# nikhilTkur/Multigrid_Nikhil_C-

Hardware: AMD Instinct MI355X
Metric: fine_grid_stencil_updates_per_sec (higher is better)
Workload: dtype f64

## Files before the change

### multigrid_nikhil_c-_amd/csrc/mgx.hip

```cpp

#include "../../include/mgx.h"
#include "mgx_bottom.hpp"
#include "mgx_kernels.hpp"
#include "mgx_launch.hpp"
#include "mgx_var.hpp"
#include "mgx_galerkin.hpp"
#include "mgx_opdep.hpp"
#include "mgx_cheby.hpp"
#include "mgx_line.hpp"
#include "mgx_colour.hpp"
#include "mgx_small.hpp"
#include "mgx_krylov.hpp"
#include "mgx_refine.hpp"
#include "mgx_refine_gcr.hpp"
#include "mgx_multi.hpp"
#include "mgx_eig.hpp"
#include "mgx_eig_many.hpp"
#include "mgx_theta.hpp"
#include "mgx_newton.hpp"
#include "mgx_dist_plan.hpp"

#include <chrono>
#include <unistd.h>
#include <cmath>
// ... 370 lines not shown
}

int lambda_update(mgx_solver* s, Level& l)
{
    if (l.f64) launch_lambda_max<double>(var_level<double>(l), s->partial, s->partial_cap, s->sum_dev, s->stream);
    else launch_lambda_max<float>(var_level<float>(l), s->partial, s->partial_cap, s->sum_dev, s->stream);
    HIPCHK(s, hipGetLastError());
    HIPCHK(s, hipMemcpyAsync(s->sum_host, s->sum_dev, sizeof(double), hipMemcpyDeviceToHost, s->stream));
    HIPCHK(s, hipStreamSynchronize(s->stream));
    l.lambda_g = *s->sum_host;
    return MGX_OK;
}

template <typename T> LineLevel<T> line_level(const Level& l)
{
    return LineLevel<T>{op9_of<T>(l), l.nine, l.N, l.pitch, (T*)l.line_m[0], (T*)l.line_g[0], (T*)l.line_m[1], (T*)l.line_g[1],
                        (T*)l.line_hf, (T*)l.line_hb, l.line_R};
}

int line_update(mgx_solver* s, Level& l)
{
    if (!s->line_dirs) return MGX_OK;
    HIPCHK(s, hipMemsetAsync(s->line_flag, 0, sizeof(int), s->stream));
    for (int d = 0; d < 2; ++d) {
        if (!(s->line_dirs & (1 << d))) continue;
        if (l.f64) launch_line_factor<double>(line_level<double>(l), d, s->line_flag, s->stream);
        else launch_line_factor<float>(line_level<float>(l), d, s->line_flag, s->stream);
    }
    HIPCHK(s, hipGetLastError());
    int flag = 0;
    HIPCHK(s, hipMemcpyAsync(&flag, s->line_flag, sizeof(int), hipMemcpyDeviceToHost, s->stream));
    HIPCHK(s, hipStreamSynchronize(s->stream));
    if (flag)
        return s->fail(MGX_ERR_INVALID, "MGX_SMOOTHER_LINE: zero or non-finite pivot in the tridiagonal factorisation of level " +
                                            std::to_string(l.L) + ", direction " + ((flag & 1) ? "x" : "y"));
    return MGX_OK;
}

template <typename T>
void build_splitting(mgx_solver* s, const Level& l)
{
    const dim3 blk(256), grd((l.N + 1 + 255) / 256, l.N + 1);
    with_point_count(l.nine, [&](auto nq) {
        hipLaunchKernelGGL((k_var_build_jacobi<T, decltype(nq)::value>), grd, blk, 0, s->stream, op9_of<T>(l), out9(jac9_of<T>(l)), l.N, l.pitch,
                           (T)s->cfg.omega);
    });
}
template <typename T>
void build_bottom_inverse(mgx_solver* s, const Level& l)
{
    const int n = l.N - 1, NN = n * n;
    with_point_count(l.nine, [&](auto nq) {
        hipLaunchKernelGGL((k_var_dense_fill<T, decltype(nq)::value>), dim3((NN + 255) / 256, NN), dim3(256), 0, s->stream, s->var_M, s->var_inv,
                           op9_of<T>(l), n, l.pitch);
    });
    gj_invert(s, NN);
}

template <typename T>
int var_build_t(mgx_solver* s, Level& l)
{
    build_splitting<T>(s, l);
    if (l.L == s->cfg.coarsest_level && s->cfg.bottom == MGX_BOTTOM_EXACT) build_bottom_inverse<T>(s, l);
    HIPCHK(s, hipGetLastError());
    HIPCHK(s, hipStreamSynchronize(s->stream));
    if (int rc = lambda_update(s, l)) return rc;
    if (int rc = line_update(s, l)) { l.stencil_set = false; operator_changed(s); return rc; }
    l.stencil_set = true;
    operator_changed(s);
    return MGX_OK;
}
int var_build(mgx_solver* s, Level& l) { return l.f64 ? var_build_t<double>(s, l) : var_build_t<float>(s, l); }

template <typename T> Wt8<T> wt8_of(const Level& c)
{
    Wt8<T> w;
    for (int x = 0; x < 8; ++x) w.w[x] = (const T*)c.wt[x];
    return w;
}
template <typename T> Wt8Out<T> wt8_out(const Level& c)
{
    Wt8Out<T> w;
    for (int x = 0; x < 8; ++x) w.w[x] = (T*)c.wt[x];
    return w;
}

inline bool opdep(const mgx_solver* s) { return s->galerkin && s->gal_built && s->transfer == MGX_TRANSFER_OPERATOR; }

template <typename T>
int galerkin_build_t(mgx_solver* s, int transfer)
{
    const int lo = s->cfg.coarsest_level, hi = s->cfg.finest_level;
    const T rscale = (s->cfg.restrict_mode == MGX_RESTRICT_FW16) ? (T)0.25 : (T)1;
    if (transfer == MGX_TRANSFER_OPERATOR)
        for (int lv = lo; lv < hi; ++lv)
            for (void*& p : s->lv[lv].wt) {
                if (p) continue;
                if (hipMalloc(&p, s->lv[lv].bytes) != hipSuccess) return s->fail(MGX_ERR_ALLOC, "hipMalloc failed for the prolongation's weight arrays");
                HIPCHK(s, hipMemsetAsync(p, 0, s->lv[lv].bytes, s->stream));
            }
    for (int lv = hi; lv > lo; --lv) {
        const Level& f = s->lv[lv];
        const Level& c = s->lv[lv - 1];
        const Launch g = make_launch(c.N, VecOf<T>::W, c.N - 1, 1);
        const dim3 grd(g.blocks), blk(kBlock);
        with_point_count(f.nine, [&](auto nq) {
            constexpr bool CORNERS = decltype(nq)::value == 9;
            if (transfer == MGX_TRANSFER_OPERATOR) {
                hipLaunchKernelGGL((k_opdep_weights<T, CORNERS>), grd, blk, 0, s->stream, op9_of<T>(f), wt8_out<T>(c), c.N, f.pitch, c.pitch, g.strips);
                hipLaunchKernelGGL((k_galerkin_rap_opdep<T, CORNERS>), grd, blk, 0, s->stream, op9_of<T>(f), wt8_of<T>(c), out9(op9_of<T>(c)), c.N,
                                   f.pitch, c.pitch, g.strips, rscale);
            }
            else hipLaunchKernelGGL((k_galerkin_rap<T, CORNERS>), grd, blk, 0, s->stream, op9_of<T>(f), out9(op9_of<T>(c)), c.N, f.pitch, c.pitch,
                                    g.strips, rscale);
        });
    }
    for (int lv = lo; lv <= hi; ++lv) build_splitting<T>(s, s->lv[lv]);
    if (s->cfg.bottom == MGX_BOTTOM_EXACT) build_bottom_inverse<T>(s, s->lv[lo]);
    HIPCHK(s, hipGetLastError());
    HIPCHK(s, hipStreamSynchronize(s->stream));
    for (int lv = lo; lv <= hi; ++lv)
        if (int rc = lambda_update(s, s->lv[lv])) return rc;
    for (int lv = lo; lv <= hi; ++lv)
        if (int rc = line_update(s, s->lv[lv])) {
            for (int c = lo; c < hi; ++c) s->lv[c].stencil_set = false;
            s->gal_built = false;
            operator_changed(s);
            return rc;
        }
    for (int lv = lo; lv <= hi; ++lv) s->lv[lv].stencil_set = true;
    s->gal_built = true;
    s->transfer = transfer;
    operator_changed(s);
    return MGX_OK;
}

void galerkin_invalidate(mgx_solver* s)
{
    s->rx.set = false;
    for (int lv = s->cfg.coarsest_level; lv < s->cfg.finest_level; ++lv) s->lv[lv].stencil_set = false;
    s->lv[s->cfg.finest_level].stencil_set = true;
    s->gal_built = false;
    operator_changed(s);
}

int var_ready(mgx_solver* s, int lo, int hi)
{
    if (!s->var) return MGX_OK;
    if (s->galerkin && !s->gal_built)
        return s->fail(MGX_ERR_STATE, s->lv[s->cfg.finest_level].stencil_set ? "Galerkin hierarchy not built (mgx_build_galerkin)"
                                                                             : "finest operator not set (mgx_set_stencil / mgx_set_coefficient / mgx_set_stencil9 / mgx_set_tensor)");
    for (int l = lo; l <= hi; ++l)
        if (!s->lv[l].stencil_set)
            return s->fail(MGX_ERR_STATE, "operator of level " + std::to_string(l) + " not set (mgx_set_stencil / mgx_set_coefficient)");
    return MGX_OK;
}

struct MultiSet { int act[MGX_MAX_RHS]; int m; };
constexpr int kOwn = -1;
constexpr MultiSet kOwnSet{{kOwn}, 1};
inline bool own(const MultiSet& a) { return a.act[0] == kOwn; }

inline MultiSet multi_all(int nrhs)
{
    MultiSet a{};
    for (int j = 0; j < nrhs; ++j) a.act[a.m++] = j;
    return a;
}

enum Slot { kU, kTmp, kB, kR };
inline void*& slot(mgx_solver* s, int level, int c, Slot which)
{
    if (c == kOwn) {
        Level& l = s->lv[level];
        void** const own_slots[] = {&l.u, &l.tmp, &l.b, &l.r};
        return *own_slots[which];
    }
    auto& w = s->multi.lv[level];
    void** const columns[] = {w.u, w.tmp, w.b, w.r};
    return columns[which][c];
}

template <typename T> struct SetPtrs { T* p[MGX_MAX_RHS]; };
template <typename T> SetPtrs<T> set_ptrs(mgx_solver* s, int level, const MultiSet& a, Slot which)
{
    SetPtrs<T> o{};
    for (int j = 0; j < a.m; ++j) o.p[j] = (T*)slot(s, level, a.act[j], which);
    return o;
}

template <typename T>
void smooth_var_t(mgx_solver* s, int level, const MultiSet& a, int mu)
{
    const T om = (T)s->cfg.omega;
    const T rc = (T)(1.0 - (double)om);
    const VarLevel<T> v = var_level<T>(s->lv[level]);
    for (int i = 0; i < mu; ++i) {
        launch_jacobi_var<T>(v, a.m, set_ptrs<const T>(s, level, a, kU).p, set_ptrs<const T>(s, level, a, kB).p, set_ptrs<T>(s, level, a, kTmp).p,
                             rc, om, s->stream);
        for (int j = 0; j < a.m; ++j) std::swap(slot(s, level, a.act[j], kU), slot(s, level, a.act[j], kTmp));
    }
    s->last_smooth_launches = mu;
}

template <typename T>
void smooth_cheby_t(mgx_solver* s, Level& l, int mu)
{
    const T om = (T)s->cfg.omega;
    const T rc = (T)(1.0 - (double)om);
    const std::vector<ChebyStep> st = cheby_scalars(s->cfg.omega, l.lambda_g, mu);
    const VarLevel<T> cl = var_level<T>(l);
    for (int i = 0; i < mu; ++i) {
        launch_cheby<T>(cl, (const T*)l.u, (const T*)l.b, (T*)l.tmp, (T*)l.cheb, i == 0, rc, om, (T)st[i].a, (T)st[i].c, s->stream);
        std::swap(l.u, l.tmp);
    }
    s->last_smooth_launches = mu;
}

template <typename T>
void smooth_line_t(mgx_solver* s, Level& l, int mu)
{
    const LineLevel<T> ll = line_level<T>(l);
    int launches = 0;
    for (int i = 0; i < mu; ++i) launches += launch_line_sweep<T>(ll, (T*)l.u, (const T*)l.b, s->line_dirs, s->stream);
    s->last_smooth_launches = launches;
}

template <typename T>
void smooth_colour_t(mgx_solver* s, Level& l, int mu, bool reverse)
{
    const ColourLevel<T> cl{op9_of<T>(l), (const T*)l.J[0], l.nine, l.N, l.pitch};
    const bool fused = s->gs_fused && !l.nine && gs_fused_level(l.N);
    int launches = 0;
    for (int i = 0; i < mu; ++i) {
        if (fused) {
            launch_gs_rb<T>(cl, (const T*)l.u, (const T*)l.b, (T*)l.tmp, reverse, s->stream);
            std::swap(l.u, l.tmp);
            ++launches;
        } else {
            launches += launch_gs_colours<T>(cl, (T*)l.u, (const T*)l.b, reverse, s->stream);
        }
    }
    s->last_smooth_launches = launches;
}

void smooth_var(mgx_solver* s, int level, const MultiSet& a, int mu, bool post = false)
{
    Level& l = s->lv[level];
    if (s->colour) {
        const bool reverse = s->colour == 2 && post;
        if (l.f64) smooth_colour_t<double>(s, l, mu, reverse); else smooth_colour_t<float>(s, l, mu, reverse);
    }
    else if (s->line_dirs) { if (l.f64) smooth_line_t<double>(s, l, mu); else smooth_line_t<float>(s, l, mu); }
    else if (s->cfg.smoother == MGX_SMOOTHER_CHEBYSHEV) { if (l.f64) smooth_cheby_t<double>(s, l, mu); else smooth_cheby_t<float>(s, l, mu); }
    else if (l.f64) smooth_var_t<double>(s, level, a, mu);
    else smooth_var_t<float>(s, level, a, mu);
}

template <typename T, int MODE>
void residual_var_t(mgx_solver* s, const Level& l, const MultiSet& a, const T* const* u, const T* const* b, T* const* out)
{
    double *part[MGX_MAX_RHS] = {}, *sums[MGX_MAX_RHS] = {};
    for (int j = 0; j < a.m; ++j) {
        const int c = a.act[j];
        part[j] = c == kOwn ? s->partial : s->multi.part[c];
        sums[j] = c == kOwn ? s->sum_dev : s->multi.sums + c;
    }
    launch_residual_var<T, MODE>(var_level<T>(l), a.m, u, b, out, part, sums, s->stream);
}

template <typename T, int MODE>
void residual_set(mgx_solver* s, int level, const MultiSet& a)
{
    residual_var_t<T, MODE>(s, s->lv[level], a, set_ptrs<const T>(s, level, a, kU).p, set_ptrs<const T>(s, level, a, kB).p,
                            MODE ? nullptr : set_ptrs<T>(s, level, a, kR).p);
}

template <int MODE>
void residual_level(mgx_solver* s, const Level& l, const void* u, const void* b, void* out)
{
    with_float_type(l.f64, [&](auto tag) {
        using T = decltype(tag);
        const T* const uu = (const T*)u;
        const T* const bb = (const T*)b;
        T* const oo = (T*)out;
        if (s->var) residual_var_t<T, MODE>(s, l, kOwnSet, &uu, &bb, &oo);
        else launch_residual<T, MODE>((const T*)u, (const T*)b, out, MODE ? 0 : l.pitch, MODE ? s->partial : nullptr, MODE ? s->sum_dev : nullptr,
                                      1.0, l.N, l.pitch, 1, l.N, s->rows_per_chunk, s->stream, MODE ? s->partial_cap : -1, l.rows);
    });
}

template <typename T, int SM, int AR>
int fold_block(const FuseCfg& fc, const BlockReq& q, T* u, const T* b, T* tmp, long pitch, double omega, const mgx_slab* c,
               const T* coarse_e, T* coarse_b, T* coarse_zero, int crow_lo, int crow_hi, int restrict_mode, double* partial,
               hipStream_t st, int* flips)
{
    std::vector<Pass> plan;
    if (!fold_plan(fc, q, &plan)) return -1;
    const int N = q.N, row0 = q.row0;
    const JacobiCoef<T> jc = jacobi_coef<T>(omega);
    FoldArgs fa;
    fa.restrict_mode = restrict_mode;
    fa.partial = partial;
    fa.win.row_first = std::max(row0, 0);
    fa.win.row_last = std::min(row0 + q.rows - 1, N);
    fa.win.crow_first = 0; fa.win.crow_last = -1; fa.win.emit_lo = 0; fa.win.emit_hi = 0;
    if (c) {
        fa.cpitch = level_pitch(c->level, c->dtype);
        fa.win.crow_first = std::max(c->row0, 0);
        fa.win.crow_last = std::min(c->row0 + c->rows - 1, N / 2);
        fa.win.emit_lo = std::max(c->row0 + crow_lo, 1);
        fa.win.emit_hi = std::min(c->row0 + crow_hi, N / 2);
        const long cback = (long)c->row0 * fa.cpitch;
        if (coarse_e) fa.coarse_e = coarse_e - cback;
        if (coarse_b) fa.coarse_b = coarse_b - cback;
        if (coarse_zero) fa.coarse_zero = coarse_zero - cback;
    }
    const long back = (long)row0 * pitch;
    T* src = u; T* dst = tmp;
    int blocks = 0;
    for (const Pass& p : plan) {
        if (p.hi > p.lo) {
            const int lo = p.lo - row0, hi = p.hi - row0;
            fa.row_lo = p.lo; fa.row_hi = p.hi;
            fa.zero_in = p.zero_in ? 1 : 0;
            int rc = 0;
            if (p.kind == PASS_JACOBI)
                rc = launch_jacobi<T>(src, b, dst, N, pitch, lo, hi, omega, p.R, st, q.rows, AR) ? -1 : 0;
            else if (p.kind == PASS_RBGS)
                launch_rbgs<T>(src, b, dst, N, pitch, lo, hi, row0 & 1, -row0, N - row0, p.R, st);
            else if (p.kind == PASS_FUSED)
                rc = launch_fused<T, SM, AR>(p.K, src, b, dst, N, pitch, lo, hi, jc.c0, jc.c1, -row0, N - row0, row0 & 1, p.R, st,
                                             q.rows, fa.zero_in) ? 0 : -1;
            else if (p.kind == PASS_FOLDED)
                rc = with_stages(p.pre, p.post, [&](auto s) {
                    using S = decltype(s);
                    if constexpr (S::PRE || S::POST)
                        return launch_cycle<T, S::PRE, S::POST, SM, AR>(p.K, src - back, b - back, dst - back, fa, N, pitch, jc.c0, jc.c1, p.R, st);
                    else
                        return -1;
                });
            else
                rc = launch_tile_pass<T, SM, AR>(src - back, b - back, dst - back, fa, N, pitch, jc.c0, jc.c1, p.K, p.R, p.pre, p.post, st);
            if (rc < 0) return -1;
            if (p.post == 2) blocks = rc;
        }
        std::swap(src, dst);
    }
    *flips = (int)plan.size();
    return blocks;
}

bool fold_eligible(const mgx_solver* s, const Level& l, int mu, bool pre = false, int post = 1, bool zero_in = false)
{
    if (!s->fold || mu < 1 || mu > 64) return false;
    if (s->var || (post == 1 && s->cfg.restrict_mode >= MGX_RESTRICT_INJECT)) return false;
    const int per = (s->cfg.smoother == MGX_SMOOTHER_RBGS) ? 2 : 1;
    if (!tile_level(s, l) && (l.N < s->fuse.min_n || s->fuse.kmax < per)) return false;
    std::vector<Pass> plan;
    return fold_plan(s->fuse, level_req(s, l, mu, pre, post, zero_in, 0), &plan);
}

bool zero_in_ok(const mgx_solver* s, int level)
{
    if (!s->use_zero_in || level <= s->cfg.coarsest_level) return false;
    return fold_eligible(s, s->lv[level], s->cfg.mu1, false, 1, true);
}

bool smooth_folded(mgx_solver* s, int level, int mu, bool pre, int post, bool zero_in = false, bool coarse_zero_in = false)
{
    Level& l = s->lv[level];
    if (!fold_eligible(s, l, mu, pre, post)) return false;
    const bool fine = (level == s->cfg.finest_level);
    const bool rbgs = (s->cfg.smoother == MGX_SMOOTHER_RBGS);
    if (!l.f64 && !rbgs && mu == 10 && l.N > s->fuse.tile_max_n && post == 2 && pre &&
        cycle_k_supported(mu, false, false, 0, pre, s->fuse.arith) && !cycle_k_supported(mu, false, false, post, pre, s->fuse.arith))
        post = 0;
    {
        Prof p(s, fine ? MGX_PROF_SMOOTH_FINE : MGX_PROF_COARSE, mu);
        const Level& c = s->lv[level - 1];
        const int dt = l.f64 ? MGX_DTYPE_F64 : MGX_DTYPE_F32;
        const mgx_slab cs{level - 1, dt, c.rows, 0, s->cfg.arith};
        void* czero = (post == 1 && coarse_zero_in) ? nullptr : c.u;
        const BlockReq q = level_req(s, l, mu, pre, post, zero_in, env_int("MGX_ROWS", 0));
        int launches = 0;
        const int nb = with_kernel_set(l.f64, s->cfg.smoother, s->fuse.arith, [&](auto k) {
            using K = decltype(k);
            using T = typename K::T;
            return fold_block<T, K::SM, K::AR>(s->fuse, q, (T*)l.u, (const T*)l.b, (T*)l.tmp, l.pitch, s->cfg.omega, &cs,
                                               pre ? (const T*)c.u : nullptr, post == 1 ? (T*)c.b : nullptr, (T*)czero, 1, c.N,
                                               s->cfg.restrict_mode, s->partial, s->stream, &launches);
        });
        if (nb < 0) return false;
        if (launches & 1) std::swap(l.u, l.tmp);
        p.set(launches, mu);
        if (post == 2) s->norm_blocks_ready = nb;
    }
    if (fine) s->fine_updates += (double)mu * (double)(l.N - 1) * (double)(l.N - 1);
    return true;
}

void smooth_t(mgx_solver* s, Level& l, int mu)
{
    int launches = 0;
    with_kernel_set(l.f64, s->cfg.smoother, s->fuse.arith, [&](auto k) {
        using K = decltype(k);
        using T = typename K::T;
        (void)fold_block<T, K::SM, K::AR>(s->fuse, level_req(s, l, mu, false, 0, false, s->rows_per_chunk), (T*)l.u, (const T*)l.b,
                                          (T*)l.tmp, l.pitch, s->cfg.omega, nullptr, nullptr, nullptr, nullptr, 0, 0, 0, nullptr,
                                          s->stream, &launches);
    });
    s->last_smooth_launches = launches;
    if (launches & 1) std::swap(l.u, l.tmp);
}

void smooth(mgx_solver* s, int level, int mu, bool post = false, const MultiSet& a = kOwnSet, double* fu = nullptr)
{
    if (mu <= 0) return;
    Level& l = s->lv[level];
    const bool fine = (level == s->cfg.finest_level);
    Prof p(s, fine ? MGX_PROF_SMOOTH_FINE : MGX_PROF_COARSE, mu, own(a));
    if (s->var) smooth_var(s, level, a, mu, post);
    else smooth_t(s, l, mu);
    p.set(s->last_smooth_launches, mu);
    if (!fine) return;
    const double updates = (double)(s->line_dirs == 3 ? 2 * mu : mu) * (double)(l.N - 1) * (double)(l.N - 1);
    if (own(a)) s->fine_updates += updates;
    else if (fu) for (int j = 0; j < a.m; ++j) fu[a.act[j]] += updates;
}

void restrict_level(mgx_solver* s, int level, bool fused, bool zero_guess, const MultiSet& a = kOwnSet)
{
    Level& f = s->lv[level];
    Level& c = s->lv[level - 1];
    const bool fine = (level == s->cfg.finest_level);
    Prof p(s, fine ? MGX_PROF_RESTRICT_FINE : MGX_PROF_COARSE, 1, own(a));
    const int rpc = s->rows_per_chunk;
    const int mode = s->cfg.restrict_mode;
    with_float_type(f.f64, [&](auto tag) {
        using T = decltype(tag);
        const SetPtrs<const T> uf = set_ptrs<const T>(s, level, a, kU), bf = set_ptrs<const T>(s, level, a, kB);
        const SetPtrs<T> cb = set_ptrs<T>(s, level - 1, a, kB);
        const SetPtrs<T> cz = zero_guess ? set_ptrs<T>(s, level - 1, a, kU) : SetPtrs<T>{};
        if (opdep(s)) {
            const Launch g = make_launch(c.N, VecOf<T>::W, c.N - 1, 1);
            const T rscale = (mode == MGX_RESTRICT_FW16) ? (T)0.25 : (T)1;
            const dim3 grd(g.blocks), blk(kBlock);
            if (!fused) hipLaunchKernelGGL((k_restrict_opdep<T, 0>), grd, blk, 0, s->stream, uf.p[0], bf.p[0], op9_of<T>(f), wt8_of<T>(c), cb.p[0],
                                           cz.p[0], c.N, f.pitch, c.pitch, g.strips, rscale);
            else with_point_count(f.nine, [&](auto nq) {
                constexpr int MODE = decltype(nq)::value == 9 ? 2 : 1;
                if (a.m == 1) hipLaunchKernelGGL((k_restrict_opdep<T, MODE>), grd, blk, 0, s->stream, uf.p[0], bf.p[0], op9_of<T>(f), wt8_of<T>(c),
                                                 cb.p[0], cz.p[0], c.N, f.pitch, c.pitch, g.strips, rscale);
                else with_count<kMultiMax, 2>(a.m, [&](auto kc) {
                    constexpr int K = decltype(kc)::value;
                    hipLaunchKernelGGL((k_restrict_opdep_multi<T, MODE, K>), grd, blk, 0, s->stream, columns_in<K>(uf.p), columns_in<K>(bf.p),
                                       op9_of<T>(f), wt8_of<T>(c), columns_out<K>(cb.p), columns_out<K>(cz.p), c.N, f.pitch, c.pitch, g.strips, rscale);
                });
            });
            return;
        }
        const bool grid_residual = fused && (s->var || mode >= MGX_RESTRICT_INJECT);
        if (grid_residual) {
            if (s->var) residual_set<T, 0>(s, level, a);
            else residual_level<0>(s, f, f.u, f.b, f.r);
        }
        const SetPtrs<const T> src = grid_residual ? set_ptrs<const T>(s, level, a, kR) : bf;
        for (int j = 0; j < a.m; ++j) {
            if (mode >= MGX_RESTRICT_INJECT) {
                const double w = (mode == MGX_RESTRICT_INJECT4) ? 4.0 : 1.0;
                const dim3 blk(256), grd((c.N + 255) / 256, c.N - 1);
                hipLaunchKernelGGL((k_restrict_inject<T>), grd, blk, 0, s->stream, src.p[j], cb.p[j], cz.p[j], c.N, f.pitch, c.pitch, (T)w);
            } else {
                launch_restrict<T>(uf.p[j], src.p[j], cb.p[j], cz.p[j], f.N, f.pitch, c.pitch, 1, c.N, 0, mode, fused && !grid_residual, rpc, s->stream);
            }
        }
    });
}

void prolong_level(mgx_solver* s, int level, bool add, const MultiSet& a = kOwnSet)
{
    Level& f = s->lv[level];
    Level& c = s->lv[level - 1];
    const bool fine = (level == s->cfg.finest_level);
    Prof p(s, fine ? MGX_PROF_PROLONG_FINE : MGX_PROF_COARSE, 1, own(a));
    with_float_type(f.f64, [&](auto tag) {
        using T = decltype(tag);
        const SetPtrs<T> v = set_ptrs<T>(s, level, a, kU);
        const SetPtrs<const T> e = set_ptrs<const T>(s, level - 1, a, kU);
        if (opdep(s)) launch_prolong_opdep<T>(a.m, add, v.p, e.p, wt8_of<T>(c), c.N, f.pitch, c.pitch, s->stream);
        else for (int j = 0; j < a.m; ++j) launch_prolong<T>(v.p[j], e.p[j], f.N, f.pitch, c.pitch, 1, f.N, 0, add, s->rows_per_chunk, s->stream);
    });
}

void bottom_solve(mgx_solver* s, const MultiSet& a = kOwnSet)
{
    const int level = s->cfg.coarsest_level;
    Level& l = s->lv[level];
    Prof p(s, (l.L == s->cfg.finest_level) ? MGX_PROF_SMOOTH_FINE : MGX_PROF_COARSE, 4, own(a));
    const int n = l.N - 1;
    with_float_type(l.f64, [&](auto tag) {
        using T = decltype(tag);
        const SetPtrs<const T> b = set_ptrs<const T>(s, level, a, kB);
        const SetPtrs<T> u = set_ptrs<T>(s, level, a, kU);
        if (s->var) launch_var_dense_solve<T>(s->var_inv, a.m, b.p, u.p, n, l.pitch, s->stream);
        else s->bottom.solve<T>(b.p[0], u.p[0], l.pitch, s->stream);
    });
}

int zero_u(mgx_solver* s, int level, const MultiSet& a = kOwnSet)
{
    for (int j = 0; j < a.m; ++j) HIPCHK(s, hipMemsetAsync(slot(s, level, a.act[j], kU), 0, s->lv[level].bytes, s->stream));
    return MGX_OK;
}

bool descend(mgx_solver* s, int level, bool zero_in_here, const MultiSet& a = kOwnSet, double* fu = nullptr)
{
    const bool zin_next = own(a) && zero_in_ok(s, level - 1);
    if (!own(a) || !smooth_folded(s, level, s->cfg.mu1, false, 1, zero_in_here, zin_next)) {
        if (zero_in_here) (void)zero_u(s, level, a);
        smooth(s, level, s->cfg.mu1, false, a, fu);
        restrict_level(s, level, true, !zin_next, a);
    }
    return zin_next;
}

void ascend(mgx_solver* s, int level, int post, const MultiSet& a = kOwnSet, double* fu = nullptr)
{
    if (!own(a) || !smooth_folded(s, level, s->cfg.mu2, true, post)) {
        prolong_level(s, level, true, a);
        smooth(s, level, s->cfg.mu2, true, a, fu);
    }
}

void vcycle(mgx_solver* s, int level, bool zero_in_here = false, int post_top = 0, int kind = -1, const MultiSet& a = kOwnSet,
            double* fu = nullptr);

bool small_level(const mgx_solver* s, int level, const MultiSet& a)
{
    if (!own(a) || !s->small_visit || s->cycle == MGX_CYCLE_V || !s->galerkin || !s->gal_built) return false;
    if (s->cfg.smoother != MGX_SMOOTHER_JACOBI) return false;
    if (level <= s->cfg.coarsest_level || level >= s->cfg.finest_level) return false;
    const Level& l = s->lv[level];
    return l.nine && l.N <= s->small_max_n;
}

void small_visit(mgx_solver* s, int level, bool ascend, bool descend)
{
    Level& f = s->lv[level];
    Level& c = s->lv[level - 1];
    Prof p(s, MGX_PROF_COARSE, 1);
    with_float_type(f.f64, [&](auto tag) {
        using T = decltype(tag);
        SmallVisit<T> a;
        a.u = (T*)f.u; a.b = (const T*)f.b;
        a.a = op9_of<T>(f); a.r = jac9_of<T>(f); a.dinv = (const T*)f.J[0];
        a.cu = (T*)c.u; a.cb = (T*)c.b;
        a.w = wt8_of<T>(c);
        a.N = f.N; a.pitch = f.pitch; a.cpitch = c.pitch;
        a.ascend = ascend; a.descend = descend; a.mu1 = s->cfg.mu1; a.mu2 = s->cfg.mu2;
        a.opdep = opdep(s);
        a.omega = (T)s->cfg.omega;
        a.rc = (T)(1.0 - (double)a.omega);
        const bool fw16 = s->cfg.restrict_mode == MGX_RESTRICT_FW16;
        a.rscale = fw16 ? (T)0.25 : (T)1;
        a.wgt = fw16 ? (T)0.0625 : (T)0.25;
        launch_small_visit<T>(a, s->stream);
    });
    p.set(1, (ascend ? s->cfg.mu2 : 0) + (descend ? s->cfg.mu1 : 0));
}

void coarse_visits(mgx_solver* s, int level, bool zero_in_here, int kind, const MultiSet& a = kOwnSet, double* fu = nullptr)
{
    const bool twice = kind != MGX_CYCLE_V && level > s->cfg.coarsest_level;
    const int second = kind == MGX_CYCLE_F ? MGX_CYCLE_V : kind;
    if (twice && small_level(s, level, a)) {
        small_visit(s, level, false, true);
        coarse_visits(s, level - 1, false, kind);
        small_visit(s, level, true, true);
        coarse_visits(s, level - 1, false, second);
        small_visit(s, level, true, false);
        return;
    }
    vcycle(s, level, zero_in_here, 0, kind, a, fu);
    if (twice) vcycle(s, level, false, 0, second, a, fu);
}

void vcycle(mgx_solver* s, int level, bool zero_in_here, int post_top, int kind, const MultiSet& a, double* fu)
{
    if (kind < 0) kind = s->cycle;
    if (level == s->cfg.coarsest_level) {
        if (s->cfg.bottom == MGX_BOTTOM_EXACT) {
            bottom_solve(s, a);
        } else {
            smooth(s, level, s->cfg.mu1, false, a, fu);
            smooth(s, level, s->cfg.mu2, true, a, fu);
        }
        return;
    }
    if (small_level(s, level, a)) {
        small_visit(s, level, false, true);
        coarse_visits(s, level - 1, false, kind);
        small_visit(s, level, true, false);
        return;
    }
    const bool zin_next = descend(s, level, zero_in_here, a, fu);
// ... 1840 lines not shown
```

### multigrid_nikhil_c-_amd/csrc/mgx_geom.hpp

```cpp
#pragma once

#if defined(__HIPCC__)
#define MGX_GEOM_HD __host__ __device__ __forceinline__
#else
#define MGX_GEOM_HD inline
#endif

namespace mgx {

constexpr int kGeomWavesPerBlock = 4;
constexpr int kGeomCusPerXcd = 32;
constexpr int kGeomResidentBlocks = 512;

struct CycleGeom {
    int R, Re, Rl;
    int Rf;
    int chunks, chunks_e;
    int row_last0;
    int RB, n_tall, n_short;
    long waves;
    int blocks;
};

struct CTile { int strip, r0, r1; bool active; };

MGX_GEOM_HD int geom_min(int a, int b) { return a < b ? a : b; }

MGX_GEOM_HD CTile cycle_tile_at(int block, int wave, int grid, int strips, int chunks, int chunks_e, int R, int Re, int row_lo,
                                int row_hi, int row_last0, int Rl, int RB, int n_tall, int n_short, int Rf)
{
    const int per_xcd = grid >> 3;
    const int xcd = block & 7;
    const int nth = block >> 3;
    const int si = strips - 2;
    CTile t;
    t.strip = 0; t.r0 = 0; t.r1 = 0; t.active = false;
    if (row_last0 != 0) {
        const int n_edge = 3 * si + 2 * chunks_e;
        int e = -1, m = -1, s = -1;
        if (n_tall > 0) {
            const int n_f = n_edge + n_tall * si, n_s = n_short * si;
            const int pf = (n_f + 7) >> 3, ps = (n_s + 7) >> 3;
            if (nth < kGeomCusPerXcd) {
                const int lw = nth * kGeomWavesPerBlock + wave;
                const int f = xcd * pf + lw;
                if (lw < pf && f < n_f) { if (f < n_edge) e = f; else m = f - n_edge; }
            } else {
                const int lw = (nth - kGeomCusPerXcd) * kGeomWavesPerBlock + wave;
                if (lw < ps && xcd * ps + lw < n_s) s = xcd * ps + lw;
            }
        } else {
            const int n_mid = (chunks - 3) * si;
            const int pe = (n_edge + 7) >> 3, pm = (n_mid + 7) >> 3;
            const int lw = nth * kGeomWavesPerBlock + wave;
            if (lw < pe) { if (xcd * pe + lw < n_edge) e = xcd * pe + lw; }
            else if (lw - pe < pm && xcd * pm + (lw - pe) < n_mid) m = xcd * pm + (lw - pe);
        }
        if (e >= 0) {
            t.active = true;
            if (e < 3 * si) {
                const int which = e / si;
                t.strip = 1 + (e - which * si);
                t.r0 = which == 0 ? row_lo : (which == 1 ? row_last0 : row_last0 + Rl);
                t.r1 = which == 0 ? row_lo + Rf : (which == 1 ? row_last0 + Rl : row_hi);
            } else {
                const int k = e - 3 * si;
                const int chunk = k >> 1;
                t.strip = (k & 1) ? strips - 1 : 0;
                t.r0 = row_lo + chunk * Re;
                t.r1 = geom_min(t.r0 + Re, row_hi);
            }
        } else if (m >= 0) {
            const int chunk = m / si;
            t.active = true;
            t.strip = 1 + (m - chunk * si);
            t.r0 = row_lo + Rf + chunk * R;
            t.r1 = geom_min(t.r0 + R, row_last0);
        } else if (s >= 0) {
            const int chunk = s / si;
            t.active = true;
            t.strip = 1 + (s - chunk * si);
            t.r0 = row_lo + Rf + n_tall * R + chunk * RB;
            t.r1 = geom_min(t.r0 + RB, row_last0);
        }
        t.active = t.active && t.r0 < t.r1;
        return t;
    }
    const int b = xcd * per_xcd + (xcd >= 4 ? per_xcd - 1 - nth : nth);
    const long g = (long)b * kGeomWavesPerBlock + wave;
    const long n_int = si > 0 ? (long)chunks * si : 0;
    if (g < n_int) {
        const int chunk = (int)(g / si);
        t.strip = 1 + (int)(g - (long)chunk * si);
        t.r0 = row_lo + chunk * R;
        t.r1 = geom_min(t.r0 + R, row_hi);
        t.active = t.r0 < t.r1;
    } else {
        const long e = g - n_int;
        int chunk;
        if (si > 0) { chunk = (int)(e >> 1); t.strip = (e & 1) ? strips - 1 : 0; }
        else { chunk = (int)(e / strips); t.strip = (int)(e - (long)chunk * strips); }
        t.r0 = row_lo + chunk * Re;
        t.r1 = geom_min(t.r0 + Re, row_hi);
        t.active = chunk < chunks_e && t.r0 < row_hi;
    }
    return t;
}


inline int trip_rows(int R, int extra, int trip, int step)
{
    int best = -1;
    for (int r = R; r < R + 2 * trip; r += step) {
        const int m = (r + extra) % trip;
        if (m == 0) return r;
        if (m == trip - 1 && best < 0) best = r;
    }
    return best < 0 ? R : best;
}

inline int edge_rows_pct(int R, int extra, int trip, int pct)
{
    const double frac = 0.01 * (double)pct;
    const int k = (int)(frac * (double)(R + extra) / (double)trip + 0.5);
    const int Re = R - k * trip;
    return Re >= trip ? Re : (R >= 2 * trip ? trip : R);
}

struct GeomKnobs {
    int edge_short = 1;
    int edge_pct = 23;
    int last_pct = 38;
    int min_chunk = 16;
    int min_rounds = 1;
    int min_rounds_rows = 1024;
    int pair = 1;
    int pair_ratio = 130;
    int pair_max_rows = 640;
    int pair_min_rows = 150;
};

inline int geom_blocks(const CycleGeom& g, int strips)
{
    int blocks = (int)(((g.waves + kGeomWavesPerBlock - 1) / kGeomWavesPerBlock + 7) / 8 * 8);
    if (g.row_last0 != 0) {
        const int si = strips - 2;
        const int n_edge = 3 * si + 2 * g.chunks_e;
        if (g.n_tall > 0) {
            const int ps = (g.n_short * si + 7) / 8;
            blocks = 8 * (kGeomCusPerXcd + (ps + kGeomWavesPerBlock - 1) / kGeomWavesPerBlock);
        } else {
            const int pe = (n_edge + 7) / 8, pm = ((g.chunks - 3) * si + 7) / 8;
            blocks = 8 * ((pe + pm + kGeomWavesPerBlock - 1) / kGeomWavesPerBlock);
        }
    }
    return blocks;
}

inline CycleGeom cycle_geom(int row_lo, int row_hi, int strips, int R, int Re, int Rl, int Rf = -1)
{
    const int rows = row_hi - row_lo;
    if (Rf < 0) Rf = Re;
    CycleGeom g;
    g.R = R; g.Re = Re; g.Rl = Rl; g.Rf = Rf; g.RB = 0; g.n_tall = 0; g.n_short = 0;
    g.chunks_e = (rows + Re - 1) / Re;
    if ((Re >= R && Rf >= R && Rl >= R) || rows <= Rf + 2 * Rl + 2 || strips < 3) {
        g.R = (Re >= R) ? R : Re; g.Re = g.R; g.Rl = g.R; g.Rf = g.R;
        g.row_last0 = 0;
        g.chunks = g.chunks_e = (rows + g.R - 1) / g.R;
    } else {
        const int last = row_hi - Rl + ((row_hi - Rl - row_lo) & 1);
        g.row_last0 = last - Rl;
        g.chunks = 3 + (g.row_last0 - (row_lo + Rf) + R - 1) / R;
    }
    g.waves = strips > 2 ? (long)g.chunks * (strips - 2) + 2L * g.chunks_e : (long)g.chunks_e * strips;
    g.blocks = geom_blocks(g, strips);
    return g;
}

inline bool cycle_geom_paired(int row_lo, int row_hi, int strips, int extra, int trip, const GeomKnobs& kn, bool top_edge, bool bot_edge,
                              CycleGeom* out)
{
    const int rows = row_hi - row_lo;
    const int si = strips - 2;
    if (si < 1) return false;
    const int slots = kGeomCusPerXcd * kGeomWavesPerBlock;
    for (int rb = trip_rows(kn.min_chunk, extra, trip, 2); rb <= kn.pair_max_rows; rb += trip) {
        const int steps_b = (rb + extra + trip - 1) / trip * trip;
        const int steps_a = (int)(((long)steps_b * kn.pair_ratio / 100 + trip - 1) / trip) * trip;
        const int ra = (steps_a - extra) & ~1;
        if (ra > kn.pair_max_rows) break;
        if (ra <= rb) continue;
        const int re = edge_rows_pct(ra, extra, trip, kn.edge_pct), rl = bot_edge ? edge_rows_pct(ra, extra, trip, kn.last_pct) : ra;
        const int rf = top_edge ? re : ra;
        if (rows <= rf + 2 * rl + 2 + rb) continue;
        const int chunks_e = (rows + re - 1) / re;
        const int n_edge = 3 * si + 2 * chunks_e;
        const int last = row_hi - rl + ((row_hi - rl - row_lo) & 1);
        const int row_last0 = last - rl;
        const int mid = row_last0 - (row_lo + rf);
        if (mid < rb) continue;
        const int nt_max = (8 * slots - 7 - n_edge) / si, ns_max = (8 * slots - 7) / si;
        if (nt_max < 1 || ns_max < 1) continue;
        if ((long)nt_max * ra + (long)ns_max * rb < mid) continue;
        if (rb < kn.pair_min_rows) return false;
        int nt = (int)((double)mid * ((double)nt_max * ra / ((double)nt_max * ra + (double)ns_max * rb)) / ra + 0.5);
        if (nt > nt_max) nt = nt_max;
        while (nt > 0 && (long)nt * ra > mid - rb) --nt;
        int ns = nt > 0 ? (mid - nt * ra + rb - 1) / rb : ns_max + 1;
        while (ns > ns_max && nt < nt_max && (long)(nt + 1) * ra <= mid - rb) { ++nt; ns = (mid - nt * ra + rb - 1) / rb; }
        if (nt < 1 || ns > ns_max) continue;
        const int pf = (n_edge + nt * si + 7) / 8, ps = (ns * si + 7) / 8;
        if (pf > slots || ps > slots) continue;
        CycleGeom g;
        g.R = ra; g.Re = re; g.Rl = rl; g.Rf = rf; g.RB = rb; g.n_tall = nt; g.n_short = ns;
        g.chunks_e = chunks_e; g.row_last0 = row_last0; g.chunks = 3 + nt + ns;
        g.waves = (long)g.chunks * si + 2L * chunks_e;
        g.blocks = geom_blocks(g, strips);
        if (g.blocks > kGeomResidentBlocks) continue;
        *out = g;
        return true;
    }
    return false;
}

inline CycleGeom cycle_geom_pick(int row_lo, int row_hi, int strips, int extra, int trip, int R, bool auto_rows, bool deep,
                                 const GeomKnobs& kn, bool top_edge = true, bool bot_edge = true)
{
    if (R & 1) ++R;
    R = trip_rows(R, extra, trip, 2);
    CycleGeom g = cycle_geom(row_lo, row_hi, strips, R, R, R);
    if (!deep) return g;
    auto shaped = [&](int r) {
        return cycle_geom(row_lo, row_hi, strips, r, kn.edge_short ? edge_rows_pct(r, extra, trip, kn.edge_pct) : r,
                          (kn.edge_short && bot_edge) ? edge_rows_pct(r, extra, trip, kn.last_pct) : r,
                          (kn.edge_short && top_edge) ? edge_rows_pct(r, extra, trip, kn.edge_pct) : r);
    };
    if (!auto_rows) return kn.edge_short ? shaped(R) : g;
    if (kn.pair && kn.edge_short && strips >= 3) {
        CycleGeom p;
        if (cycle_geom_paired(row_lo, row_hi, strips, extra, trip, kn, top_edge, bot_edge, &p)) return p;
    }
    bool found = false;
    for (int m = (row_hi - row_lo >= kn.min_rounds_rows ? kn.min_rounds : 1); m <= 64 && !found; ++m) {
        for (int r = trip_rows(kn.min_chunk, extra, trip, 2); r <= 204; r += trip) {
            const CycleGeom c = shaped(r);
            if (c.waves <= 2048L * m && c.blocks <= kGeomResidentBlocks * m) { g = c; found = true; break; }
        }
    }
    return g;
}

constexpr int kTileWideWaves = 8;

struct TileWideGeom {
    int He, Hx;
    int TH, TW;
    int tiles_y, tiles_x;
};

MGX_GEOM_HD TileWideGeom tile_wide_geom(int N, int row_lo, int row_hi, int He, int W, int RW)
{
    TileWideGeom g;
    g.He = He;
    g.Hx = (He + W - 1) / W * W;
    g.TH = kTileWideWaves * RW - 2 * He;
    g.TW = 64 * W - 2 * g.Hx;
    g.tiles_y = (g.TH > 0 && row_hi > row_lo) ? (row_hi - row_lo + g.TH - 1) / g.TH : 0;
    g.tiles_x = g.TW > 0 ? (N + g.TW - 1) / g.TW : 0;
    return g;
}

MGX_GEOM_HD int tile_wide_rw(int N, int short_max_n) { return N <= short_max_n ? 8 : 10; }

}
```

### multigrid_nikhil_c-_amd/csrc/mgx_kernels.hpp

```cpp
#pragma once

#include <hip/hip_runtime.h>
#include "mgx_geom.hpp"
#include "mgx_phase_trace.hpp"
#include <stdint.h>
#include <type_traits>

namespace mgx {

template <int B, int E, typename F> __device__ __forceinline__ void static_for(F&& f)
{
    if constexpr (B < E) {
        f(std::integral_constant<int, B>{});
        static_for<B + 1, E>(f);
    }
}

constexpr int kWave = 64;
constexpr int kBlock = 256;
constexpr int kWavesPerBlock = kBlock / kWave;
constexpr int kOutLanes = kWave - 2;

template <typename T> struct VecOf;
template <> struct VecOf<double> { using type = double2; static constexpr int W = 2; };
// ... 510 lines not shown
            MGX_FSTEP(0, y); MGX_FSTEP(1, y + 1); MGX_FSTEP(2, y + 2);
        }
    }
#undef MGX_FSTEP
}

template <typename T, int K, int SM = 0, int AR = 0>
__global__ void __launch_bounds__(kBlock)
k_jacobi_fused(const T* __restrict__ vin, const T* __restrict__ rhs, T* __restrict__ vout,
               int N, long pitch, int row_lo, int row_hi, int R, int strips, int chunks,
               T c0, T c1, int bnd_lo, int bnd_hi, int row_parity, int rows_alloc, int zero_in)
{
    constexpr int W = VecOf<T>::W;
    constexpr int HL = (K + W - 1) / W;
    constexpr int OUT = kWave - 2 * HL;
    const Tile t = wave_tile(strips, chunks);
    if (!t.active) return;
    const int lane = threadIdx.x & 63;
    const int vx = t.strip * OUT - HL + lane;
    const long col = (long)vx * W;
    const bool ld = (vx >= 0) && (col + W <= pitch);
    const bool st = (lane >= HL) && (lane < kWave - HL) && (vx < N / W);
    const int r0 = row_lo + t.chunk * R;
    const int r1 = min(r0 + R, row_hi);
    const T* pv = vin + col;
    const T* pb = rhs + col;
    T* po = vout + col;
    const int rd_lo = max(bnd_lo, 0), rd_hi = min(bnd_hi, rows_alloc - 1);
    const int vx0 = t.strip * OUT - HL;
    const bool interior = (vx0 >= 1) && ((long)(vx0 + kWave) * W < N) &&
                          (r0 - K - 1 > bnd_lo) && (r0 - K - 1 >= 0) &&
                          (r1 + K + trip_steps<T>() + kPrefetch < bnd_hi) && (r1 + K + trip_steps<T>() + kPrefetch <= rows_alloc - 1);
    FastOut fo;
    fo.rb = max(r0 - K - 1, rd_lo);
    fo.crb = 0;
    fo.pitch_bytes = (unsigned)(pitch * (long)sizeof(T));
    fo.cpitch_bytes = 0;
    const unsigned f_bytes = rsrc_bytes(fo.rb, rows_alloc - 1, fo.pitch_bytes);
    const long f_at = (long)fo.rb * pitch;
    fo.out = make_rsrc(vout + f_at, f_bytes);
    fo.in = make_rsrc(vin + f_at, f_bytes);
    fo.rhs = make_rsrc(rhs + f_at, f_bytes);
    fo.cb = fo.out; fo.cz = fo.out; fo.ce = fo.out;
    fo.lane_off = (unsigned)(col * (long)sizeof(T));
    fo.clane_off = 0;
    if (interior) {
        if (zero_in) fused_body<T, K, SM, false, true, AR>(pv, pb, po, pitch, col, N, r0, r1, true, st, c0, c1, bnd_lo, bnd_hi, rd_lo, rd_hi, row_parity, true, fo);
        else fused_body<T, K, SM, false, false, AR>(pv, pb, po, pitch, col, N, r0, r1, true, st, c0, c1, bnd_lo, bnd_hi, rd_lo, rd_hi, row_parity, false, fo);
    } else {
        fused_body<T, K, SM, true, false, AR>(pv, pb, po, pitch, col, N, r0, r1, ld, st, c0, c1, bnd_lo, bnd_hi, rd_lo, rd_hi, row_parity, zero_in != 0, fo);
    }
}

template <int K, int W> constexpr int fused_out_lanes() { return kWave - 2 * ((K + W - 1) / W); }

__device__ __forceinline__ double2 residual_vec(const double2& up, const double2& cur, const double2& dn, const double2& bb)
{
    const double l = from_left(cur.y), r = from_right(cur.x);
    double2 o;
    o.x = bb.x - (-nbr(up.x, l, cur.y, dn.x) + 4.0 * cur.x);
    o.y = bb.y - (-nbr(up.y, cur.x, r, dn.y) + 4.0 * cur.y);
    return o;
}
__device__ __forceinline__ float4 residual_vec(const float4& up, const float4& cur, const float4& dn, const float4& bb)
{
    const NbrPairs t = nbr_pairs(up, cur, dn);
    const f32x2 p0 = {cur.x, cur.y}, p1 = {cur.z, cur.w}, b0 = {bb.x, bb.y}, b1 = {bb.z, bb.w};
    const f32x2 o0 = b0 - (-t.t0 + 4.f * p0);
    const f32x2 o1 = b1 - (-t.t1 + 4.f * p1);
    return make_float4(o0.x, o0.y, o1.x, o1.y);
}

template <typename T, int MODE>
__global__ void __launch_bounds__(kBlock)
k_residual(const T* __restrict__ vin, const T* __restrict__ rhs, void* __restrict__ out, long pitch_out,
           double* __restrict__ partial, double inv_scale,
           int N, long pitch, int row_lo, int row_hi, int R, int strips, int chunks, int rows_alloc)
{
    using V = typename VecOf<T>::type;
    constexpr int W = VecOf<T>::W;
    __shared__ double wsum[kWavesPerBlock];
    const Tile t = wave_tile(strips, chunks);
    double acc = 0.0;
    if (t.active) {
        const Cols c = lane_cols<W>(t.strip, N, pitch);
        const int r0 = row_lo + t.chunk * R;
        const int r1 = min(r0 + R, row_hi);
        const T* pv = vin + c.col;
        const T* pb = rhs + c.col;
        auto has = [&](int y) { return c.ld && y >= 0 && y < rows_alloc; };
        V up = vload<V>(pv + (long)(r0 - 1) * pitch, has(r0 - 1));
        V cur = vload<V>(pv + (long)r0 * pitch, has(r0));
        for (int r = r0; r < r1; ++r) {
            const V dn = vload<V>(pv + (long)(r + 1) * pitch, has(r + 1));
            const V bb = vload<V>(pb + (long)r * pitch, has(r));
            V o = residual_vec(up, cur, dn, bb);
            mask_cols(o, c.col, N);
            if (MODE == 0) {
                vstore<V>(reinterpret_cast<T*>(out) + c.col + (long)r * pitch, o, c.st);
            } else {
                if (c.st) {
                    if constexpr (W == 2) acc += (double)o.x * (double)o.x + (double)o.y * (double)o.y;
                    else acc += ((double)o.x * (double)o.x + (double)o.y * (double)o.y) +
                                ((double)o.z * (double)o.z + (double)o.w * (double)o.w);
                }
                if constexpr (MODE == 2 && W == 2) {
                    float2 f = make_float2((float)(o.x * inv_scale), (float)(o.y * inv_scale));
                    if (c.st) *reinterpret_cast<float2*>(reinterpret_cast<float*>(out) + c.col + (long)r * pitch_out) = f;
                }
            }
            up = cur; cur = dn;
        }
    }
    if (MODE != 0) {
        for (int off = 32; off > 0; off >>= 1) acc += __shfl_down(acc, off, kWave);
        if ((threadIdx.x & 63) == 0) wsum[threadIdx.x >> 6] = acc;
        __syncthreads();
        if (threadIdx.x == 0) {
            double s = 0.0;
            for (int w = 0; w < kWavesPerBlock; ++w) s += wsum[w];
            partial[blockIdx.x] = s;
        }
    }
}

constexpr int kReduceThreads = 1024;
static __global__ void __launch_bounds__(kReduceThreads) k_reduce_partials(const double* __restrict__ partial, int n, double* __restrict__ out)
{
    __shared__ double wsum[kReduceThreads / kWave];
    double a0 = 0.0, a1 = 0.0, a2 = 0.0, a3 = 0.0;
    int i = threadIdx.x;
    for (; i + 3 * kReduceThreads < n; i += 4 * kReduceThreads) {
        a0 += partial[i];
        a1 += partial[i + kReduceThreads];
        a2 += partial[i + 2 * kReduceThreads];
        a3 += partial[i + 3 * kReduceThreads];
    }
    for (; i < n; i += kReduceThreads) a0 += partial[i];
    double acc = (a0 + a1) + (a2 + a3);
    for (int off = 32; off > 0; off >>= 1) acc += __shfl_down(acc, off, kWave);
    if ((threadIdx.x & 63) == 0) wsum[threadIdx.x >> 6] = acc;
    __syncthreads();
    if (threadIdx.x == 0) {
        double s = 0.0;
        for (int w = 0; w < kReduceThreads / kWave; ++w) s += wsum[w];
        out[0] = s;
    }
}

struct ReduceSum { __device__ __forceinline__ double operator()(double a, double b) const { return a + b; } };
struct ReduceMax { __device__ __forceinline__ double operator()(double a, double b) const { return b > a ? b : a; } };
template <int NW, typename OP>
__device__ __forceinline__ void block_reduce(double acc, double* wsum, double* __restrict__ out, OP op)
{
    for (int off = 32; off > 0; off >>= 1) acc = op(acc, __shfl_down(acc, off, kWave));
    if ((threadIdx.x & 63) == 0) wsum[threadIdx.x >> 6] = acc;
    __syncthreads();
    if (threadIdx.x == 0) {
        double s = 0.0;
        for (int w = 0; w < NW; ++w) s = op(s, wsum[w]);
        *out = s;
    }
}

template <typename T> struct Trip { T l, c, r; };

template <typename T> __device__ __forceinline__ T restrict_fw_value(const Trip<T>& top, const Trip<T>& mid, const Trip<T>& bot, T wgt)
{
    T corners = top.l + top.r; corners = corners + bot.l; corners = corners + bot.r;
    T edges = mid.l + mid.r; edges = edges + top.c; edges = edges + bot.c;
    return wgt * ((corners + (T)2 * edges) + (T)4 * mid.c);
}
template <typename T> __device__ __forceinline__ T prolong_edge_value(T a, T b) { return (T)0.5 * (a + b); }
template <typename T> __device__ __forceinline__ T prolong_centre_value(T nw, T sw, T ne, T se) { return (T)0.25 * (((nw + sw) + ne) + se); }

template <typename T, bool FUSED>
__global__ void __launch_bounds__(kBlock)
k_restrict(const T* __restrict__ vin, const T* __restrict__ rhs, T* __restrict__ coarse, T* __restrict__ coarse_zero,
           int N, long pitch, long cpitch, int crow_lo, int crow_hi, int fine_row_off,
           int R, int strips, int chunks, T wgt)
{
    using V = typename VecOf<T>::type;
    constexpr int W = VecOf<T>::W;
    constexpr int CW = W / 2;
    const Tile t = wave_tile(strips, chunks);
    if (!t.active) return;
    const Cols c = lane_cols<W>(t.strip, N, pitch);
    const int I0 = crow_lo + t.chunk * R;
    const int I1 = min(I0 + R, crow_hi);
    const T* pv = vin + c.col;
    const T* pb = rhs + c.col;
    const long ccol = c.col / 2;
    const int NC = N / 2;

    auto row_plain = [&](int y) -> V { V o = vload<V>(pb + (long)y * pitch, c.ld); mask_cols(o, c.col, N); return o; };

    V up, cur, dn;
    int yf = 2 * I0 + fine_row_off - 1;
    if (FUSED) {
        up = vload<V>(pv + (long)(yf - 1) * pitch, c.ld);
        cur = vload<V>(pv + (long)yf * pitch, c.ld);
    }
    auto next_field = [&](int y) -> V {
        if (FUSED) {
            dn = vload<V>(pv + (long)(y + 1) * pitch, c.ld);
            const V bb = vload<V>(pb + (long)y * pitch, c.ld);
            V o = residual_vec(up, cur, dn, bb);
            mask_cols(o, c.col, N);
            up = cur; cur = dn;
            return o;
        } else {
            return row_plain(y);
        }
    };
    auto trips = [&](const V& f, Trip<T>* tr) {
        const T l = from_left(last(f));
        if constexpr (W == 2) { tr[0] = {l, f.x, f.y}; }
        else { tr[0] = {l, f.x, f.y}; tr[1] = {f.y, f.z, f.w}; }
    };

    Trip<T> top[CW], mid[CW], bot[CW];
    { const V f = next_field(yf); trips(f, top); }
    for (int I = I0; I < I1; ++I) {
        const int y = 2 * I + fine_row_off;
        { const V f = next_field(y); trips(f, mid); }
        { const V f = next_field(y + 1); trips(f, bot); }
        T o[CW];
#pragma unroll
        for (int k = 0; k < CW; ++k) {
            o[k] = restrict_fw_value(top[k], mid[k], bot[k], wgt);
            if (ccol + k == 0 || ccol + k >= NC) o[k] = (T)0;
        }
        if (c.st) {
            T* pc = coarse + (long)I * cpitch + ccol;
            if constexpr (CW == 1) { pc[0] = o[0]; }
            else { *reinterpret_cast<float2*>(pc) = make_float2((float)o[0], (float)o[1]); }
            if (coarse_zero) {
                T* pz = coarse_zero + (long)I * cpitch + ccol;
                if constexpr (CW == 1) { pz[0] = (T)0; }
                else { *reinterpret_cast<float2*>(pz) = make_float2(0.f, 0.f); }
            }
        }
#pragma unroll
        for (int k = 0; k < CW; ++k) top[k] = bot[k];
    }
}

template <typename T, bool ADD>
__global__ void __launch_bounds__(kBlock)
k_prolong(T* __restrict__ v, const T* __restrict__ coarse, int N, long pitch, long cpitch,
          int row_lo, int row_hi, int fine_row_off, int R, int strips, int chunks)
{
    using V = typename VecOf<T>::type;
    constexpr int W = VecOf<T>::W;
    constexpr int CW = W / 2;
    const Tile t = wave_tile(strips, chunks);
    if (!t.active) return;
    const Cols c = lane_cols<W>(t.strip, N, pitch);
    const int r0 = row_lo + t.chunk * R;
    const int r1 = min(r0 + R, row_hi);
    T* pv = v + c.col;
    const long ccol = c.col / 2;
    const bool cld = c.ld && (ccol + CW < cpitch);

    auto crow = [&](int I, T* e) {
        const T* p = coarse + (long)I * cpitch + ccol;
#pragma unroll
        for (int k = 0; k <= CW; ++k) e[k] = cld ? p[k] : (T)0;
    };
    for (int r = r0; r < r1; ++r) {
        const int y = r - fine_row_off;
        const int I = y >> 1;
        T a[CW + 1], b2[CW + 1];
        crow(I, a);
        V add;
        T o[W];
        if ((y & 1) == 0) {
#pragma unroll
            for (int k = 0; k < CW; ++k) { o[2 * k] = a[k]; o[2 * k + 1] = prolong_edge_value(a[k], a[k + 1]); }
        } else {
            crow(I + 1, b2);
#pragma unroll
            for (int k = 0; k < CW; ++k) {
                o[2 * k] = prolong_edge_value(a[k], b2[k]);
                o[2 * k + 1] = prolong_centre_value(a[k], b2[k], a[k + 1], b2[k + 1]);
            }
        }
        if constexpr (W == 2) add = make_double2(o[0], o[1]);
        else add = make_float4(o[0], o[1], o[2], o[3]);
        mask_cols(add, c.col, N);
        if (ADD) {
            const V old = vload<V>(pv + (long)r * pitch, c.st);
            if constexpr (W == 2) { add.x = old.x + add.x; add.y = old.y + add.y; }
            else { add.x = old.x + add.x; add.y = old.y + add.y; add.z = old.z + add.z; add.w = old.w + add.w; }
        }
        vstore<V>(pv + (long)r * pitch, add, c.st);
    }
}

template <int K, int POST> constexpr int cycle_halo_cols() { return K + (POST == 1 ? 2 : (POST == 2 ? 1 : 0)); }
template <int K, int POST, int W> constexpr int cycle_out_lanes() { return kWave - 2 * ((cycle_halo_cols<K, POST>() + W - 1) / W); }

template <typename T, int CW> struct CycleState {
    T ct[CW], tc[CW], em[CW], mc[CW];
    T ea[CW + 1];
    double acc;
};

struct CycleWin {
    int row_first, row_last;
    int crow_first, crow_last;
    int emit_lo, emit_hi;
};

struct CycleArgs {
    long cpitch; int NC;
    int r0, r1, y_end;
    bool zero_in;
    CycleWin win;
};

template <typename T, int CW> struct PreFetch { T a[CW + 1], b[CW + 1]; };

template <typename T, bool EDGE>
__device__ __forceinline__ void
coarse_loads(PreFetch<T, VecOf<T>::W / 2>& pe, int y, const T* __restrict__ coarse_e, long cpitch, long ccol, int N, bool cld,
             const CycleWin& win, const FastOut& fo)
{
    constexpr int CW = VecOf<T>::W / 2;
    const int I = y >> 1;
    if constexpr (!EDGE) {
        const int Ia = min(max(I, win.crow_first), win.crow_last), Ib = min(max(I + 1, win.crow_first), win.crow_last);
        const unsigned srow_a = (unsigned)(Ia - fo.crb) * fo.cpitch_bytes, srow_b = (unsigned)(Ib - fo.crb) * fo.cpitch_bytes;
#pragma unroll
        for (int k = 0; k <= CW; ++k) pe.a[k] = bload1_s((T*)nullptr, fo.ce, fo.clane_off + (unsigned)(k * sizeof(T)), srow_a);
#pragma unroll
        for (int k = 0; k <= CW; ++k) pe.b[k] = bload1_s((T*)nullptr, fo.ce, fo.clane_off + (unsigned)(k * sizeof(T)), srow_b);
    } else {
        const bool cl = cld && y > 0 && y < N && I >= win.crow_first && I + (y & 1) <= win.crow_last;
        const bool cl2 = cl && (y & 1);
        const unsigned at = (unsigned)(I - fo.crb) * fo.cpitch_bytes + fo.clane_off;
#pragma unroll
        for (int k = 0; k <= CW; ++k) pe.a[k] = bload1((T*)nullptr, fo.ce, cl ? at + (unsigned)(k * sizeof(T)) : kOobOffset);
#pragma unroll
        for (int k = 0; k <= CW; ++k) pe.b[k] = bload1((T*)nullptr, fo.ce, cl2 ? at + fo.cpitch_bytes + (unsigned)(k * sizeof(T)) : kOobOffset);
    }
}

template <typename T, bool EDGE>
__device__ __forceinline__ void
coarse_row(T (&e)[VecOf<T>::W / 2 + 1], int I, bool cld, const CycleWin& win, const FastOut& fo)
{
    constexpr int CW = VecOf<T>::W / 2;
    if constexpr (!EDGE) {
        const int Ic = min(max(I, win.crow_first), win.crow_last);
        const unsigned srow = (unsigned)(Ic - fo.crb) * fo.cpitch_bytes;
#pragma unroll
        for (int k = 0; k <= CW; ++k) e[k] = bload1_s((T*)nullptr, fo.ce, fo.clane_off + (unsigned)(k * sizeof(T)), srow);
    } else {
        const bool ok = cld && I >= win.crow_first && I <= win.crow_last;
        const unsigned at = (unsigned)(I - fo.crb) * fo.cpitch_bytes + fo.clane_off;
#pragma unroll
        for (int k = 0; k <= CW; ++k) e[k] = bload1((T*)nullptr, fo.ce, ok ? at + (unsigned)(k * sizeof(T)) : kOobOffset);
    }
}

template <typename T, bool EDGE, bool ZIN = false>
__device__ __forceinline__ void
cycle_loads(typename VecOf<T>::type& in, typename VecOf<T>::type& bn, int y,
            const T* __restrict__ pv, const T* __restrict__ pb, long pitch, int N, int y_end, bool ld, bool zero_in,
            const CycleWin& win, const FastOut& fo)
{
    using V = typename VecOf<T>::type;
    if constexpr (!EDGE) {
        const int yi = min(y, win.row_last), yb = max(min(y - 1, win.row_last), win.row_first);
        if constexpr (ZIN) in = vzero((V*)nullptr);
        else in = bload_s((V*)nullptr, fo.in, fo.lane_off, (unsigned)(yi - fo.rb) * fo.pitch_bytes);
        bn = bload_s((V*)nullptr, fo.rhs, fo.lane_off, (unsigned)(yb - fo.rb) * fo.pitch_bytes);
    } else {
        const bool in_ok = !zero_in && y >= win.row_first && y <= win.row_last && y < y_end;
        const bool b_ok = (y - 1) > 0 && (y - 1) < N && (y - 1) >= win.row_first && (y - 1) <= win.row_last && y <= y_end;
        in = bload((V*)nullptr, fo.in, (ld && in_ok) ? (unsigned)(y - fo.rb) * fo.pitch_bytes + fo.lane_off : kOobOffset);
        bn = bload((V*)nullptr, fo.rhs, (ld && b_ok) ? (unsigned)(y - 1 - fo.rb) * fo.pitch_bytes + fo.lane_off : kOobOffset);
    }
}

constexpr int kBRing = 12;
template <typename T, int K, int POST, int SM> constexpr bool cycle_b_in_lds() { return (sizeof(T) == 8 && K >= 8) || (sizeof(T) == 4 && K >= 10); }
static_assert(kBRing % 2 == 0, "the deep bodies' step parity needs an even trip");
template <typename T, int K, int POST, int SM> constexpr int cycle_par() { return cycle_b_in_lds<T, K, POST, SM>() ? ((1 + K + (POST ? 1 : 0)) & 1) : -1; }
template <typename T, int K, int POST, int SM> __device__ __forceinline__ int cycle_y0(int r0)
{
    constexpr int PAR = cycle_par<T, K, POST, SM>();
    const int y0 = r0 - K - (POST ? 1 : 0);
    return PAR < 0 ? y0 : y0 - ((y0 - PAR) & 1);
}
#ifndef MGX_SKEW
#define MGX_SKEW 0
#endif
#ifndef MGX_RING_AHEAD
#define MGX_RING_AHEAD 1
#endif
#ifndef MGX_PRIO_ALT
#define MGX_PRIO_ALT 0
#endif
template <typename T, int K, int PRE, int POST, int SM, int AR> constexpr int cycle_skew()
{
    if (sizeof(T) == 8 && K == 10 && PRE == 1 && POST == 0 && SM == 0 && AR == 0) return 0;
    if (sizeof(T) == 4 && K == 10 && PRE == 0 && POST == 1 && SM == 0) return 0;
    return (MGX_SKEW != 0 && cycle_b_in_lds<T, K, POST, SM>()) ? K / 2 : 0;
}
constexpr int kRawLds = 6;
#ifndef MGX_RAWQ
#define MGX_RAWQ 1
#endif
template <typename T, int K, int PRE, int POST, int SM, int AR> constexpr bool cycle_rawq();
template <typename T> struct LdsVec;
template <> struct LdsVec<double> { typedef double v __attribute__((ext_vector_type(2))); };
template <> struct LdsVec<float> { typedef float v __attribute__((ext_vector_type(4))); };
template <typename T> using lds_vec_ptr = __attribute__((address_space(3))) typename LdsVec<T>::v*;
__device__ __forceinline__ void ring_put(lds_vec_ptr<double> r, int slot, const double2& v)
{
    LdsVec<double>::v t = {v.x, v.y};
    r[slot * kWave] = t;
}
__device__ __forceinline__ double2 ring_get(lds_vec_ptr<double> r, int slot)
{
    const LdsVec<double>::v t = r[slot * kWave];
    return make_double2(t.x, t.y);
}
__device__ __forceinline__ void ring_put(lds_vec_ptr<float> r, int slot, const float4& v)
{
    LdsVec<float>::v t = {v.x, v.y, v.z, v.w};
    r[slot * kWave] = t;
}
__device__ __forceinline__ float4 ring_get(lds_vec_ptr<float> r, int slot)
{
    const LdsVec<float>::v t = r[slot * kWave];
    return make_float4(t.x, t.y, t.z, t.w);
}
constexpr int ring_slot(int m) { return ((m % kBRing) + kBRing) % kBRing; }
template <typename T, int K, int PRE, int POST, int SM, int AR> constexpr bool cycle_rawq()
{
    if (MGX_RAWQ == 0) return false;
    if (PRE != 0 || sizeof(T) != 8) return false;
    if (POST == 2 && AR == 0 && K == 10) return false;
    return cycle_b_in_lds<T, K, POST, SM>() && SM == 0 && POST != 0 && K > kRawLds && cycle_skew<T, K, PRE, POST, SM, AR>() == 0;
}
#ifndef MGX_PFD_DEEP
#define MGX_PFD_DEEP 0
#endif
template <bool BL, int POST, bool EDGE = false> constexpr int cycle_pfd()
{
    if (BL && !EDGE && MGX_PFD_DEEP > 0) return MGX_PFD_DEEP;
    return (BL && (POST == 1 || EDGE)) ? 2 : kPrefetch;
}
constexpr int kPrefetchMax = MGX_PFD_DEEP > kPrefetch ? MGX_PFD_DEEP : kPrefetch;
template <typename T, bool BL, bool EDGE, int POST> constexpr int cycle_cpfd() { return (BL && !(EDGE && POST == 0)) ? cycle_pfd<BL, POST, EDGE>() : 1; }

template <typename T, int K, int PRE, int POST, int SM, bool EDGE, int RP, bool BL, bool ZIN, int AR, int YP>
__device__ __forceinline__ void
cycle_step(typename VecOf<T>::type (&lev)[K + 1][3], typename VecOf<T>::type (&bw)[BL ? 1 : K + 1], lds_vec_ptr<T> ring,
           lds_vec_ptr<T> ring2, typename VecOf<T>::type (&rawq)[cycle_rawq<T, K, PRE, POST, SM, AR>() ? kBRing : 1],
           typename VecOf<T>::type (&nin)[kPfStages], typename VecOf<T>::type (&nbn)[kPfStages], PreFetch<T, VecOf<T>::W / 2>& pe,
           CycleState<T, VecOf<T>::W / 2>& cs, int y,
           const T* __restrict__ pv, const T* __restrict__ pb, T* __restrict__ po,
           const T* __restrict__ coarse_e, T* __restrict__ coarse_b, T* __restrict__ coarse_zero, T wgt,
           long pitch, long col, long ccol, int N, const CycleArgs& ca, bool ld, bool cld, bool st, T c0, T c1,
           const FastOut& fo)
{
    using V = typename VecOf<T>::type;
    constexpr int W = VecOf<T>::W;
    constexpr int CW = W / 2;
    constexpr int P = RP % 3;
    constexpr int S_OLD = (P + 1) % 3, S_MID = (P + 2) % 3, S_NEW = P;
    constexpr int bnd_lo = 0;
    const int bnd_hi = N;
    const int r0 = ca.r0, r1 = ca.r1;

    if constexpr (EDGE) __builtin_amdgcn_sched_barrier(0);
    V in = nin[0];
    const V bn = nbn[0];
#pragma unroll
    for (int q = 0; q + 1 < kPfStages; ++q) { nin[q] = nin[q + 1]; nbn[q] = nbn[q + 1]; }
    cycle_loads<T, EDGE, ZIN>(nin[kPfStages - 1], nbn[kPfStages - 1], y + cycle_pfd<BL, POST, EDGE>(), pv, pb, pitch, N, ca.y_end, ld, ca.zero_in, ca.win, fo);
    const ColMask cm = col_mask(col, N);
    if (PRE) {
        T o[W];
        bool row_zero = false;
        if constexpr (YP < 0) {
            T a[CW + 1], b2[CW + 1];
#pragma unroll
            for (int k = 0; k <= CW; ++k) { a[k] = pe.a[k]; b2[k] = pe.b[k]; }
            coarse_loads<T, EDGE>(pe, y + cycle_cpfd<T, BL, EDGE, POST>(), coarse_e, ca.cpitch, ccol, N, cld, ca.win, fo);
            const bool even = (y & 1) == 0;
#pragma unroll
            for (int k = 0; k < CW; ++k) {
                const T ab = a[k] + b2[k];
                const T ev1 = (T)0.5 * (a[k] + a[k + 1]);
                const T od0 = (T)0.5 * ab;
                const T od1 = (T)0.25 * ((ab + a[k + 1]) + b2[k + 1]);
                o[2 * k] = even ? a[k] : od0;
                o[2 * k + 1] = even ? ev1 : od1;
            }
        } else {
            constexpr int CPFD = cycle_cpfd<T, BL, EDGE, POST>();
            T b2[CW + 1];
            if constexpr (YP == 1) {
#pragma unroll
                for (int k = 0; k <= CW; ++k) b2[k] = pe.b[k];
            }
            if constexpr (((YP + CPFD) & 1) == 1) coarse_row<T, EDGE>(pe.b, ((y + CPFD) >> 1) + 1, cld, ca.win, fo);
#pragma unroll
            for (int k = 0; k < CW; ++k) {
                if constexpr (YP == 0) {
                    o[2 * k] = cs.ea[k];
                    o[2 * k + 1] = (T)0.5 * (cs.ea[k] + cs.ea[k + 1]);
                } else {
                    const T ab = cs.ea[k] + b2[k];
                    o[2 * k] = (T)0.5 * ab;
                    o[2 * k + 1] = (T)0.25 * ((ab + cs.ea[k + 1]) + b2[k + 1]);
                }
            }
            if constexpr (YP == 1) {
#pragma unroll
                for (int k = 0; k <= CW; ++k) cs.ea[k] = b2[k];
            }
            if constexpr (EDGE) {
                const int I = y >> 1;
                row_zero = !(y > 0 && y < N && I >= ca.win.crow_first && I + YP <= ca.win.crow_last);
            }
        }
        V add;
        if constexpr (W == 2) add = make_double2(o[0], o[1]);
        else add = make_float4(o[0], o[1], o[2], o[3]);
        if constexpr (EDGE) mask_sel(add, cm, row_zero);
        if constexpr (W == 2) { in.x = in.x + add.x; in.y = in.y + add.y; }
        else { in.x = in.x + add.x; in.y = in.y + add.y; in.z = in.z + add.z; in.w = in.w + add.w; }
    }
    constexpr bool RAWQ = cycle_rawq<T, K, PRE, POST, SM, AR>();
    constexpr bool PREMUL = (SM == 0 && POST == 0) || RAWQ;
    V b0;
    if constexpr (PREMUL) b0 = vscale(c1, bn);
    else b0 = bn;
    if constexpr (BL) {
        asm volatile("" : "+v"(ring));
        ring_put(ring, ring_slot(RP), b0);
        if constexpr (RAWQ) {
            asm volatile("" : "+v"(ring2));
            rawq[ring_slot(RP)] = ring_get(ring2, RP % kRawLds);
            ring_put(ring2, RP % kRawLds, bn);
        }
    } else {
#pragma unroll
        for (int j = K; j > 0; --j) bw[j] = bw[j - 1];
        bw[0] = b0;
    }
    constexpr int kRingAhead = MGX_RING_AHEAD;
    constexpr int SK = cycle_skew<T, K, PRE, POST, SM, AR>();
    constexpr int SKD = SK > 0 ? 1 : 0;
    constexpr int MLAST = ((POST && !RAWQ) ? K : K - 1) + SKD;
    V rq[BL ? K + 2 : 1];
    auto bwin = [&](auto jc) -> V {
        constexpr int j = decltype(jc)::value;
        if constexpr (j == 0) return b0;
        else if constexpr (BL) return rq[j];
        else return bw[j];
    };
    V dying = lev[SK][S_NEW];
    lev[0][S_NEW] = in;
    auto level = [&](auto jc, auto bc) {
        constexpr int j = decltype(jc)::value;
        constexpr bool inB = decltype(bc)::value;
        const int row = y - j - (inB ? 1 : 0);
        const V cb = bwin(std::integral_constant<int, j - 1 + (inB ? 1 : 0)>{});
        const V& lo = (inB && j == SK + 1) ? dying : lev[j - 1][S_OLD];
        const V& mi = (inB && j == SK + 1) ? lev[j - 1][S_OLD] : lev[j - 1][S_MID];
        const V& hi = (inB && j == SK + 1) ? lev[j - 1][S_MID] : lev[j - 1][S_NEW];
        V o;
        if constexpr (PREMUL) o = jacobi_vec_pre<AR>(lo, mi, hi, cb, c0, c1);
        else o = level_op<T, SM, AR>(j, lo, mi, hi, cb, c0, c1, row + (int)(col & 1));
        if constexpr (EDGE) {
            const int rw = opaque_s(row);
            mask_sel(o, cm, !(rw > bnd_lo && rw < bnd_hi));
        }
        if constexpr (j == K) {
            const unsigned at = (unsigned)(row - fo.rb) * fo.pitch_bytes + fo.lane_off;
            bstore(o, fo.out, (st && row >= r0 && row < r1) ? at : kOobOffset);
        }
        if (j < K || POST) lev[j][S_NEW] = o;
    };
    if constexpr (SK == 0) {
        if constexpr (BL) {
            static_for<1, (kRingAhead < MLAST ? kRingAhead : MLAST) + 1>([&](auto mc) {
                constexpr int m = decltype(mc)::value;
                rq[m] = ring_get(ring, ring_slot(RP - m));
            });
        }
        static_for<1, K + 1>([&](auto jc) {
            constexpr int j = decltype(jc)::value;
            if constexpr (BL && j + kRingAhead <= MLAST) {
                rq[j + kRingAhead] = ring_get(ring, ring_slot(RP - (j + kRingAhead)));
                __builtin_amdgcn_sched_barrier(0);
            }
            level(jc, std::false_type{});
        });
    } else {
        constexpr int NB = K - SK;
        constexpr int NP = SK > NB ? SK : NB;
        rq[SK + 1] = ring_get(ring, ring_slot(RP - (SK + 1)));
        static_for<1, NP + 1>([&](auto ic) {
            constexpr int i = decltype(ic)::value;
            if constexpr (i + 1 <= SK) rq[i] = ring_get(ring, ring_slot(RP - i));
            if constexpr (i + 1 <= NB) rq[SK + i + 1] = ring_get(ring, ring_slot(RP - (SK + i + 1)));
            if constexpr (POST != 0 && i == NP) rq[K + 1] = ring_get(ring, ring_slot(RP - (K + 1)));
            __builtin_amdgcn_sched_barrier(0);
            if constexpr (i <= SK) level(std::integral_constant<int, i>{}, std::false_type{});
            if constexpr (i <= NB) level(std::integral_constant<int, SK + i>{}, std::true_type{});
        });
    }
    if (POST) {
        const int rho = y - K - 1 - SKD;
        V rawb;
        if constexpr (RAWQ) rawb = rawq[ring_slot(RP - (K - kRawLds))];
        else rawb = bwin(std::integral_constant<int, K + SKD>{});
        V res = residual_vec(lev[K][S_OLD], lev[K][S_MID], lev[K][S_NEW], rawb);
        if constexpr (EDGE) {
            const int rw = opaque_s(rho);
            mask_sel(res, cm, !(rw > bnd_lo && rw < bnd_hi));
        }
        if (POST == 2) {
            double r2;
            if constexpr (W == 2) r2 = (double)res.x * (double)res.x + (double)res.y * (double)res.y;
            else r2 = ((double)res.x * (double)res.x + (double)res.y * (double)res.y) +
                      ((double)res.z * (double)res.z + (double)res.w * (double)res.w);
            cs.acc += (st && rho >= r0 && rho < r1) ? r2 : 0.0;
        } else {
            T cl[CW], cc[CW], cr[CW];
            const T l = from_left(last(res));
            if constexpr (W == 2) { cl[0] = l; cc[0] = res.x; cr[0] = res.y; }
            else { cl[0] = l; cc[0] = res.x; cr[0] = res.y; cl[1] = res.y; cc[1] = res.z; cr[1] = res.w; }
            constexpr int RHOP = YP < 0 ? -1 : ((YP + K + 1 + SKD) & 1);
            const int I = (rho - 1) >> 1;
            if constexpr (RHOP < 0) {
                const bool odd = (rho & 1) != 0;
                const bool emit = odd && (2 * I >= r0) && (2 * I < r1) && I >= ca.win.emit_lo && I < ca.win.emit_hi;
                T o[CW];
#pragma unroll
                for (int k = 0; k < CW; ++k) {
                    T corners = cs.ct[k] + cl[k]; corners = corners + cr[k];
                    const T edges = cs.em[k] + cc[k];
                    o[k] = wgt * ((corners + (T)2 * edges) + (T)4 * cs.mc[k]);
                    if constexpr (EDGE) o[k] = (ccol + k == 0 || ccol + k >= ca.NC) ? (T)0 : o[k];
                }
                {
                    const unsigned at = (st && emit) ? ((unsigned)(I - fo.crb) * fo.cpitch_bytes + fo.clane_off) : kOobOffset;
                    if constexpr (CW == 1) { bstore8(o[0], fo.cb, at); bstore8((T)0, fo.cz, at); }
                    else { bstore8(make_float2((float)o[0], (float)o[1]), fo.cb, at); bstore8(make_float2(0.f, 0.f), fo.cz, at); }
                }
#pragma unroll
                for (int k = 0; k < CW; ++k) {
                    const T lr = cl[k] + cr[k];
                    const T em = lr + cs.tc[k];
                    cs.em[k] = odd ? cs.em[k] : em;
                    cs.mc[k] = odd ? cs.mc[k] : cc[k];
                    cs.ct[k] = odd ? lr : cs.ct[k];
                    cs.tc[k] = odd ? cc[k] : cs.tc[k];
                }
            } else if constexpr (RHOP == 1) {
                auto close_row = [&](bool emit) {
                    T o[CW];
#pragma unroll
                    for (int k = 0; k < CW; ++k) {
                        T corners = cs.ct[k] + cl[k]; corners = corners + cr[k];
                        const T edges = cs.em[k] + cc[k];
                        o[k] = wgt * ((corners + (T)2 * edges) + (T)4 * cs.mc[k]);
                        if constexpr (EDGE) o[k] = (ccol + k == 0 || ccol + k >= ca.NC) ? (T)0 : o[k];
                    }
                    const unsigned at = (st && emit) ? ((unsigned)(I - fo.crb) * fo.cpitch_bytes + fo.clane_off) : kOobOffset;
                    if constexpr (CW == 1) { bstore8(o[0], fo.cb, at); bstore8((T)0, fo.cz, at); }
                    else { bstore8(make_float2((float)o[0], (float)o[1]), fo.cb, at); bstore8(make_float2(0.f, 0.f), fo.cz, at); }
                };
                close_row((2 * I >= r0) && (2 * I < r1) && I >= ca.win.emit_lo && I < ca.win.emit_hi);
#pragma unroll
                for (int k = 0; k < CW; ++k) { cs.ct[k] = cl[k] + cr[k]; cs.tc[k] = cc[k]; }
            } else {
#pragma unroll
                for (int k = 0; k < CW; ++k) { cs.em[k] = (cl[k] + cr[k]) + cs.tc[k]; cs.mc[k] = cc[k]; }
            }
        }
    }
}

template <typename T, int K, int PRE, int POST, int SM, bool EDGE, bool ZIN, int AR>
__device__ __forceinline__ double
cycle_body(const T* __restrict__ pv, const T* __restrict__ pb, T* __restrict__ po,
           const T* __restrict__ coarse_e, T* __restrict__ coarse_b, T* __restrict__ coarse_zero, T wgt,
           long pitch, long cpitch, long col, int N, int r0, int r1, bool ld, bool st, T c0, T c1, bool zero_in,
           const CycleWin& win, lds_vec_ptr<T> ring, lds_vec_ptr<T> ring2, const FastOut& fo)
{
    constexpr bool BL = cycle_b_in_lds<T, K, POST, SM>();
    constexpr bool RAWQ = cycle_rawq<T, K, PRE, POST, SM, AR>();
    using V = typename VecOf<T>::type;
    constexpr int W = VecOf<T>::W;
    constexpr int CW = W / 2;
    constexpr int EBOT = POST == 1 ? 2 : (POST == 2 ? 1 : 0);
    const V Z = vzero((V*)nullptr);
    const long ccol = col / 2;
    const bool cld = ld && (ccol + CW < cpitch);
    V lev[K + 1][3];
    V bw[BL ? 1 : K + 1];
#pragma unroll
    for (int j = 0; j <= K; ++j) { lev[j][0] = Z; lev[j][1] = Z; lev[j][2] = Z; }
#pragma unroll
    for (int j = 0; j < (BL ? 1 : K + 1); ++j) bw[j] = Z;
    if constexpr (BL) {
#pragma unroll
        for (int q = 0; q < kBRing; ++q) ring_put(ring, q, Z);
    }
    V rawq[RAWQ ? kBRing : 1];
#pragma unroll
    for (int q = 0; q < (RAWQ ? kBRing : 1); ++q) rawq[q] = Z;
    if constexpr (RAWQ) {
#pragma unroll
        for (int q = 0; q < kRawLds; ++q) ring_put(ring2, q, Z);
    }
    CycleState<T, CW> cs;
    cs.acc = 0.0;
#pragma unroll
    for (int k = 0; k < CW; ++k) cs.ct[k] = cs.tc[k] = cs.em[k] = cs.mc[k] = (T)0;
#pragma unroll
    for (int k = 0; k <= CW; ++k) cs.ea[k] = (T)0;
    CycleArgs ca;
    ca.cpitch = cpitch; ca.NC = N / 2; ca.r0 = r0; ca.r1 = r1; ca.zero_in = zero_in; ca.win = win;
    constexpr int PAR = cycle_par<T, K, POST, SM>();
    const int y0 = cycle_y0<T, K, POST, SM>(r0);
    ca.y_end = r1 + K + EBOT + (cycle_skew<T, K, PRE, POST, SM, AR>() > 0 ? 1 : 0);
    constexpr int kRound = BL ? kBRing : trip_steps<T>();
    const int steps = (ca.y_end - y0 + kRound - 1) / kRound * kRound;
    constexpr int PFD = cycle_pfd<BL, POST, EDGE>();
    V nin[PFD][kPfStages], nbn[PFD][kPfStages];
    constexpr int CPFD = cycle_cpfd<T, BL, EDGE, POST>();
    PreFetch<T, CW> pe[CPFD];
#pragma unroll
    for (int q = 0; q < CPFD; ++q) {
#pragma unroll
        for (int k = 0; k <= CW; ++k) { pe[q].a[k] = (T)0; pe[q].b[k] = (T)0; }
    }
#pragma unroll
    for (int q = 0; q < PFD; ++q)
        cycle_loads<T, EDGE, ZIN>(nin[q][0], nbn[q][0], y0 + q, pv, pb, pitch, N, ca.y_end, ld, ca.zero_in, ca.win, fo);
    if (PRE) {
        if constexpr (PAR < 0) {
#pragma unroll
            for (int q = 0; q < CPFD; ++q) coarse_loads<T, EDGE>(pe[q], y0 + q, coarse_e, cpitch, ccol, N, cld, ca.win, fo);
        } else {
            coarse_row<T, EDGE>(cs.ea, y0 >> 1, cld, ca.win, fo);
#pragma unroll
            for (int q = 0; q < CPFD; ++q)
                if (((PAR + q) & 1) == 1) coarse_row<T, EDGE>(pe[q].b, ((y0 + q) >> 1) + 1, cld, ca.win, fo);
        }
    }
#define MGX_CSTEP(RP, Y) cycle_step<T, K, PRE, POST, SM, EDGE, RP, BL, ZIN, AR, (PAR < 0 ? -1 : ((PAR + (RP)) & 1))>(lev, bw, ring, ring2, rawq, nin[(RP) % PFD], nbn[(RP) % PFD], pe[(RP) % CPFD], cs, Y, pv, pb, po, coarse_e, coarse_b, coarse_zero, wgt, pitch, col, ccol, N, ca, ld, cld, st, c0, c1, fo)
    if constexpr (BL) {
#define MGX_CTRIP(Y) do { MGX_CSTEP(0, Y); MGX_CSTEP(1, Y + 1); MGX_CSTEP(2, Y + 2); MGX_CSTEP(3, Y + 3); MGX_CSTEP(4, Y + 4); \
                          MGX_CSTEP(5, Y + 5); MGX_CSTEP(6, Y + 6); MGX_CSTEP(7, Y + 7); MGX_CSTEP(8, Y + 8); MGX_CSTEP(9, Y + 9); \
                          MGX_CSTEP(10, Y + 10); MGX_CSTEP(11, Y + 11); } while (0)
#if MGX_PRIO_ALT
        unsigned hw_id;
        asm volatile("s_getreg_b32 %0, hwreg(HW_REG_HW_ID)" : "=s"(hw_id));
        int turn = (int)(hw_id & 1u);
        for (int y = y0; y < y0 + steps; y += kBRing) {
            if (turn & 1) __builtin_amdgcn_s_setprio(1); else __builtin_amdgcn_s_setprio(0);
            turn ^= 1;
            MGX_CTRIP(y);
        }
        __builtin_amdgcn_s_setprio(0);
#else
        for (int y = y0; y < y0 + steps; y += kBRing) MGX_CTRIP(y);
#endif
#undef MGX_CTRIP
    } else if constexpr (trip_steps<T>() == 12) {
        for (int y = y0; y < y0 + steps; y += 12) {
            MGX_CSTEP(0, y); MGX_CSTEP(1, y + 1); MGX_CSTEP(2, y + 2);
            MGX_CSTEP(3, y + 3); MGX_CSTEP(4, y + 4); MGX_CSTEP(5, y + 5);
            MGX_CSTEP(6, y + 6); MGX_CSTEP(7, y + 7); MGX_CSTEP(8, y + 8);
            MGX_CSTEP(9, y + 9); MGX_CSTEP(10, y + 10); MGX_CSTEP(11, y + 11);
        }
    } else {
        for (int y = y0; y < y0 + steps; y += 3) {
            MGX_CSTEP(0, y); MGX_CSTEP(1, y + 1); MGX_CSTEP(2, y + 2);
        }
    }
#undef MGX_CSTEP
    return cs.acc;
}

template <typename T, int K, int PRE, int POST, int SM, int AR> constexpr int cycle_waves()
{
    return cycle_b_in_lds<T, K, POST, SM>() ? 2 : 1;
}
template <typename T, int K, int PRE, int POST, int SM = 0, int AR = 0>
__global__ void __launch_bounds__(kBlock, (cycle_waves<T, K, PRE, POST, SM, AR>()))
k_jacobi_cycle(const T* __restrict__ vin, const T* __restrict__ rhs, T* __restrict__ vout,
               const T* __restrict__ coarse_e,
               T* __restrict__ coarse_b, T* __restrict__ coarse_zero, T wgt,
               double* __restrict__ partial,
               int N, long pitch, long cpitch, int row_lo, int row_hi, int R, int strips, int chunks, int Re, int chunks_e,
               int row_last0, int Rl, int RB, int n_tall, int n_short, int Rf, T c0, T c1, int zero_in, CycleWin win)
{
    constexpr int W = VecOf<T>::W;
    constexpr int XC = cycle_halo_cols<K, POST>();
    constexpr int HL = (XC + W - 1) / W;
    constexpr int OUT = kWave - 2 * HL;
    constexpr int ETOP = POST ? 1 : 0;
    constexpr int EBOT = POST == 1 ? 2 : (POST == 2 ? 1 : 0);
    __shared__ double wsum[kWavesPerBlock];
    constexpr bool BL = cycle_b_in_lds<T, K, POST, SM>();
    __shared__ typename LdsVec<T>::v bring[BL ? kWavesPerBlock * kBRing * kWave : 1];
    constexpr bool RAWQ = cycle_rawq<T, K, PRE, POST, SM, AR>();
    __shared__ typename LdsVec<T>::v braw[RAWQ ? kWavesPerBlock * kRawLds * kWave : 1];
    const CTile t = cycle_tile(strips, chunks, chunks_e, R, Re, row_lo, row_hi, row_last0, Rl, RB, n_tall, n_short, Rf);
    double acc = 0.0;
#ifdef MGX_WAVE_TRACE
    const long long trace_t0 = wall_clock64();
#endif
    if (t.active) {
        const int lane = threadIdx.x & 63;
        const int wv = __builtin_amdgcn_readfirstlane(threadIdx.x >> 6);
        lds_vec_ptr<T> ring = (lds_vec_ptr<T>)&bring[BL ? (wv * kBRing * kWave + lane) : 0];
        lds_vec_ptr<T> ring2 = (lds_vec_ptr<T>)&braw[RAWQ ? (wv * kRawLds * kWave + lane) : 0];
        const int vx0 = t.strip * OUT - HL;
        const int vx = vx0 + lane;
        const long col = (long)vx * W;
        const bool ld = (vx >= 0) && (col + W <= pitch);
        const bool st = (lane >= HL) && (lane < kWave - HL) && (vx < N / W);
        const int r0 = t.r0, r1 = t.r1;
        constexpr int kRound = BL ? kBRing : trip_steps<T>();
        const int y_first = cycle_y0<T, K, POST, SM>(r0) - 1;
        constexpr int SKD = cycle_skew<T, K, PRE, POST, SM, AR>() > 0 ? 1 : 0;
        const int y_lastp = (r0 - K - ETOP) + ((r1 + K + EBOT + SKD) - (r0 - K - ETOP) + kRound - 1) / kRound * kRound + kPrefetchMax;
        const int y0c = r0 - K - ETOP, y1c = r1 + K + EBOT - 1;
        bool interior = (vx0 >= 1) && ((long)(vx0 + kWave + 1) * W < N) &&
                        (y0c > 0) && (y1c < N) && (y0c >= win.row_first) && (y1c <= win.row_last);
        interior = interior && (y_first + 1 >= win.row_first);
        if (PRE) interior = interior && (y0c >> 1) >= win.crow_first && ((y1c + 1) >> 1) <= win.crow_last;
        interior = interior && !(PRE != 0 && zero_in);
        FastOut fo;
        fo.rb = max(y_first, win.row_first);
        fo.crb = max(y_first >> 1, win.crow_first);
        fo.pitch_bytes = (unsigned)(pitch * (long)sizeof(T));
        fo.cpitch_bytes = (unsigned)(cpitch * (long)sizeof(T));
        const unsigned f_bytes = rsrc_bytes(fo.rb, win.row_last, fo.pitch_bytes);
        const unsigned c_bytes = rsrc_bytes(fo.crb, win.crow_last, fo.cpitch_bytes);
        const long f_at = (long)fo.rb * pitch, c_at = (long)fo.crb * cpitch;
        fo.out = make_rsrc(vout + f_at, f_bytes);
        fo.in = make_rsrc(vin + f_at, f_bytes);
        fo.rhs = make_rsrc(rhs + f_at, f_bytes);
        fo.ce = make_rsrc(PRE ? coarse_e + c_at : nullptr, (PRE && coarse_e) ? c_bytes : 0u);
        fo.cb = make_rsrc((POST == 1 && coarse_b) ? coarse_b + c_at : nullptr, (POST == 1 && coarse_b) ? c_bytes : 0u);
        fo.cz = make_rsrc((POST == 1 && coarse_zero) ? coarse_zero + c_at : nullptr, (POST == 1 && coarse_zero) ? c_bytes : 0u);
        fo.lane_off = (unsigned)(col * (long)sizeof(T));
        fo.clane_off = (unsigned)((col / 2) * (long)sizeof(T));
        if (interior) {
            if (PRE == 0 && zero_in)
                acc = cycle_body<T, K, PRE, POST, SM, false, PRE == 0, AR>(vin + col, rhs + col, vout + col, coarse_e, coarse_b, coarse_zero, wgt,
                                                                      pitch, cpitch, col, N, r0, r1, true, st, c0, c1, true, win, ring, ring2, fo);
            else
                acc = cycle_body<T, K, PRE, POST, SM, false, false, AR>(vin + col, rhs + col, vout + col, coarse_e, coarse_b, coarse_zero, wgt,
                                                                    pitch, cpitch, col, N, r0, r1, true, st, c0, c1, false, win, ring, ring2, fo);
        } else {
            acc = cycle_body<T, K, PRE, POST, SM, true, false, AR>(vin + col, rhs + col, vout + col, coarse_e, coarse_b, coarse_zero, wgt,
                                                        pitch, cpitch, col, N, r0, r1, ld, st, c0, c1, zero_in != 0, win, ring, ring2, fo);
        }
    }
#ifdef MGX_WAVE_TRACE
    if ((threadIdx.x & 63) == 0) {
        const int w = blockIdx.x * kWavesPerBlock + (threadIdx.x >> 6);
        if (w < (1 << 16)) {
            unsigned hw, xcc;
            asm volatile("s_getreg_b32 %0, hwreg(HW_REG_HW_ID)" : "=s"(hw));
            asm volatile("s_getreg_b32 %0, hwreg(HW_REG_XCC_ID)" : "=s"(xcc));
            g_wave_trace[w] = WaveTrace{trace_t0, wall_clock64(), t.active ? t.strip : -1, t.r0, t.r1,
                                        (int)((hw & 0xFFF0FFFFu) | ((xcc & 0xFu) << 16))};
        }
        if (w == 0) g_wave_trace_n = gridDim.x * kWavesPerBlock;
    }
#endif
    if (POST == 2) {
        for (int off = 32; off > 0; off >>= 1) acc += __shfl_down(acc, off, kWave);
        if ((threadIdx.x & 63) == 0) wsum[threadIdx.x >> 6] = acc;
        __syncthreads();
        if (threadIdx.x == 0) {
            double sum = 0.0;
            for (int w = 0; w < kWavesPerBlock; ++w) sum += wsum[w];
            partial[blockIdx.x] = sum;
        }
    }
}

constexpr int kTileBand = 14;
constexpr int kTileSY = kWavesPerBlock * kTileBand;
constexpr int kTileSX = kWave;

template <int POST> constexpr int tile_extra() { return POST == 1 ? 2 : (POST == 2 ? 1 : 0); }

template <typename T, int SM, int PRE, int POST, int AR = 0>
__global__ void __launch_bounds__(kBlock)
k_tile_smooth(const T* __restrict__ vin, const T* __restrict__ rhs, T* __restrict__ vout,
              const T* __restrict__ coarse_e, T* __restrict__ coarse_b, T* __restrict__ coarse_zero, T wgt,
              double* __restrict__ partial, int N, long pitch, long cpitch, int levels, T c0, T c1,
              int tiles_x, int zero_in, int row_lo, int row_hi, CycleWin win)
{
    constexpr int RW = kTileBand;
    __shared__ T edge[2][kWavesPerBlock][2][kWave];
    __shared__ double wsum[kWavesPerBlock];
    const int He = levels + tile_extra<POST>();
    const int TH = kTileSY - 2 * He, TW = kTileSX - 2 * He;
    const int lane = threadIdx.x & 63;
    const int wv = __builtin_amdgcn_readfirstlane(threadIdx.x >> 6);
    const int ty = blockIdx.x / tiles_x, tx = blockIdx.x - ty * tiles_x;
    const int y0 = wv * RW;
    const int gy0 = row_lo + ty * TH - He + y0;
    const int gx = 1 + tx * TW - He + lane;
    const bool colunk = gx > 0 && gx < N;
    const int NC = N / 2;

    T u[RW], b[RW];
    unsigned rowmask = 0;
#pragma unroll
    for (int i = 0; i < RW; ++i) {
        const int gy = gy0 + i;
        const bool rowok = gy > 0 && gy < N && gy >= win.row_first && gy <= win.row_last;
        if (rowok) rowmask |= 1u << i;
        const bool unk = colunk && rowok;
        const long at = (long)gy * pitch + gx;
        u[i] = (unk && !zero_in) ? vin[at] : (T)0;
        b[i] = unk ? rhs[at] : (T)0;
    }
    if (PRE) {
        const bool codd = (gx & 1) != 0;
#pragma unroll
        for (int i = 0; i < RW; ++i) {
            const int gy = gy0 + i;
            const bool rodd = (gy & 1) != 0;
            const bool unk = colunk && ((rowmask >> i) & 1u) && (gy >> 1) >= win.crow_first && (gy >> 1) + (rodd ? 1 : 0) <= win.crow_last;
            const T* e = coarse_e + (long)(gy >> 1) * cpitch + (gx >> 1);
            const T a00 = unk ? e[0] : (T)0;
            const T a01 = (unk && codd) ? e[1] : (T)0;
            const T a10 = (unk && rodd) ? e[cpitch] : (T)0;
            const T a11 = (unk && rodd && codd) ? e[cpitch + 1] : (T)0;
            const T ev = codd ? (T)0.5 * (a00 + a01) : a00;
            const T od = codd ? (T)0.25 * (((a00 + a10) + a01) + a11) : (T)0.5 * (a00 + a10);
            const T add = rodd ? od : ev;
            u[i] = unk ? u[i] + add : u[i];
        }
    }

    int buf = 0;
    auto halo_rows = [&](const T (&a)[RW], T& up, T& dn) {
        edge[buf][wv][0][lane] = a[0];
        edge[buf][wv][1][lane] = a[RW - 1];
        __syncthreads();
        up = wv > 0 ? edge[buf][wv - 1][1][lane] : (T)0;
        dn = wv < kWavesPerBlock - 1 ? edge[buf][wv + 1][0][lane] : (T)0;
        buf ^= 1;
    };
    for (int j = 1; j <= levels; ++j) {
        T up, dn;
        halo_rows(u, up, dn);
        const bool colact = colunk && lane >= j && lane < kTileSX - j;
        const int ilo = max(j - y0, 0), ihi = min(kTileSY - j - y0, RW);
        const unsigned act = ihi > ilo ? (rowmask & (((1u << (ihi - ilo)) - 1u) << ilo)) : 0u;
        T prev = up;
#pragma unroll
        for (int i = 0; i < RW; ++i) {
            const T cur = u[i];
            const T below = (i == RW - 1) ? dn : u[i + 1];
            const T l = from_left(cur), r = from_right(cur);
            const bool rowact = (act >> i) & 1u;
            if (SM == 0) {
                const T o = jac_pt<AR>(c0, cur, c1 * b[i], c1, nbr(prev, l, r, below));
                u[i] = (colact && rowact) ? o : cur;
            } else {
                const T o = (T)0.25 * (b[i] + nbr(prev, l, r, below));
                u[i] = (colact && rowact && ((gy0 + i + gx) & 1) == ((j - 1) & 1)) ? o : cur;
            }
            prev = cur;
        }
    }

    const bool colout = lane >= He && lane < He + TW && gx < N;
#pragma unroll
    for (int i = 0; i < RW; ++i) {
        const int y = y0 + i, gy = gy0 + i;
        if (y >= He && y < He + TH && gy < N && gy >= row_lo && gy < row_hi && colout) vout[(long)gy * pitch + gx] = u[i];
    }

    if (POST != 0) {
        T up, dn;
        halo_rows(u, up, dn);
        T res[RW];
        double acc = 0.0;
        T prev = up;
#pragma unroll
        for (int i = 0; i < RW; ++i) {
            const T cur = u[i];
            const T below = (i == RW - 1) ? dn : u[i + 1];
            const int y = y0 + i, gy = gy0 + i;
            const T l = from_left(cur), r = from_right(cur);
            T rr = (T)0;
            if (colunk && gy > 0 && gy < N) rr = b[i] - (-nbr(prev, l, r, below) + (T)4 * cur);
            res[i] = rr;
            if (POST == 2 && y >= He && y < He + TH && gy >= row_lo && gy < row_hi && colout) acc += (double)rr * (double)rr;
            prev = cur;
        }
        if (POST == 2) {
            for (int off = 32; off > 0; off >>= 1) acc += __shfl_down(acc, off, kWave);
            if (lane == 0) wsum[wv] = acc;
            __syncthreads();
            if (threadIdx.x == 0) {
                double sum = 0.0;
                for (int w2 = 0; w2 < kWavesPerBlock; ++w2) sum += wsum[w2];
                partial[blockIdx.x] = sum;
            }
        }
        if (POST == 1) {
            T rup, rdn;
            halo_rows(res, rup, rdn);
            const int J = gx >> 1;
            const bool cst = colout && (gx & 1) == 0 && J >= 1 && J < NC;
#pragma unroll
            for (int i = 0; i < RW; ++i) {
                const T c = res[i];
                const T n = (i == 0) ? rup : res[i - 1];
                const T s2 = (i == RW - 1) ? rdn : res[i + 1];
                const int y = y0 + i, gy = gy0 + i;
                T corners = from_left(n) + from_right(n);
                corners = corners + from_left(s2);
                corners = corners + from_right(s2);
                T edges = from_left(c) + from_right(c);
                edges = edges + n;
                edges = edges + s2;
                const T o = wgt * ((corners + (T)2 * edges) + (T)4 * c);
                if (cst && y >= He && y < He + TH && (gy & 1) == 0 && gy < N && gy >= row_lo && gy < row_hi &&
                    (gy >> 1) >= win.emit_lo && (gy >> 1) < win.emit_hi) {
                    const long at = (long)(gy >> 1) * cpitch + J;
                    coarse_b[at] = o;
                    if (coarse_zero) coarse_zero[at] = (T)0;
                }
            }
        }
    }
}

__device__ __forceinline__ double vget(const double2& v, int e) { return e == 0 ? v.x : v.y; }
__device__ __forceinline__ float vget(const float4& v, int e) { return e == 0 ? v.x : (e == 1 ? v.y : (e == 2 ? v.z : v.w)); }
__device__ __forceinline__ double2 vmake(const double (&a)[2]) { return make_double2(a[0], a[1]); }
__device__ __forceinline__ float4 vmake(const float (&a)[4]) { return make_float4(a[0], a[1], a[2], a[3]); }

template <typename T, int SM, int PRE, int POST, int AR, int RW>
__global__ void __launch_bounds__(kTileWideWaves * kWave)
k_tile_wide(const T* __restrict__ vin, const T* __restrict__ rhs, T* __restrict__ vout,
            const T* __restrict__ coarse_e, T* __restrict__ coarse_b, T* __restrict__ coarse_zero, T wgt,
            double* __restrict__ partial, int N, long pitch, long cpitch, int levels, T c0, T c1,
            int tiles_x, int zero_in, int row_lo, int row_hi, CycleWin win)
{
    using V = typename VecOf<T>::type;
    constexpr int W = VecOf<T>::W;
    constexpr int NW = kTileWideWaves;
    __shared__ V edge[2][NW][2][kWave];
    __shared__ double wsum[NW];
    MGX_PHASE_BEGIN();
    const TileWideGeom g = tile_wide_geom(N, row_lo, row_hi, levels + tile_extra<POST>(), W, RW);
    const int He = g.He, TH = g.TH, TW = g.TW;
    const int lane = threadIdx.x & 63;
    const int wv = __builtin_amdgcn_readfirstlane(threadIdx.x >> 6);
    const int ty = blockIdx.x / tiles_x, tx = blockIdx.x - ty * tiles_x;
    const int y0 = wv * RW;
    const int gy0 = row_lo + ty * TH - He + y0;
    const int cx0 = tx * TW;
    const int gx0 = cx0 - g.Hx + W * lane;
    const bool vld = gx0 >= 0 && gx0 < N;
    const bool cu0 = vld && gx0 > 0;
    bool cu[W];
#pragma unroll
    for (int e = 0; e < W; ++e) cu[e] = e == 0 ? cu0 : vld;
    const int NC = N / 2;
    MGX_PHASE_AFTER(gx0 + gy0);

    T u[RW][W], b[RW][W];
    unsigned rowmask = 0;
#pragma unroll
    for (int i = 0; i < RW; ++i) {
        const int gy = gy0 + i;
        const bool rowok = gy > 0 && gy < N && gy >= win.row_first && gy <= win.row_last;
        if (rowok) rowmask |= 1u << i;
        const long at = (long)gy * pitch + gx0;
        V uv = vzero((V*)nullptr), bv = vzero((V*)nullptr);
        if (vld && rowok) {
            bv = *reinterpret_cast<const V*>(rhs + at);
            if (!zero_in) uv = *reinterpret_cast<const V*>(vin + at);
        }
#pragma unroll
        for (int e = 0; e < W; ++e) {
            u[i][e] = cu[e] ? vget(uv, e) : (T)0;
            b[i][e] = cu[e] ? vget(bv, e) : (T)0;
        }
    }
    if (PRE) {
        constexpr int NCR = RW / 2 + 1, NCC = W / 2 + 1;
        const int kc0 = gy0 >> 1, J = gx0 >> 1;
        T cr[NCR][NCC];
#pragma unroll
        for (int k = 0; k < NCR; ++k) {
            const int cy = kc0 + k;
            const bool ok = vld && cy >= 0 && cy <= NC && cy >= win.crow_first && cy <= win.crow_last;
            const T* ep = coarse_e + (long)cy * cpitch + J;
#pragma unroll
            for (int m = 0; m < NCC; ++m) cr[k][m] = ok ? ep[m] : (T)0;
        }
        auto correct = [&](auto parity) {
            constexpr int par = decltype(parity)::value;
#pragma unroll
            for (int i = 0; i < RW; ++i) {
                const int gy = gy0 + i;
                const bool rodd = ((par + i) & 1) != 0;
                const int kr = (par + i) >> 1;
                const bool rin = ((rowmask >> i) & 1u) && (gy >> 1) >= win.crow_first && (gy >> 1) + (rodd ? 1 : 0) <= win.crow_last;
#pragma unroll
                for (int e = 0; e < W; ++e) {
                    const bool codd = (e & 1) != 0;
                    const bool unk = cu[e] && rin;
                    const T a00 = unk ? cr[kr][e >> 1] : (T)0;
                    const T a01 = (unk && codd) ? cr[kr][(e >> 1) + 1] : (T)0;
                    const T a10 = (unk && rodd) ? cr[kr + (rodd ? 1 : 0)][e >> 1] : (T)0;
                    const T a11 = (unk && rodd && codd) ? cr[kr + (rodd ? 1 : 0)][(e >> 1) + 1] : (T)0;
                    const T ev = codd ? (T)0.5 * (a00 + a01) : a00;
                    const T od = codd ? (T)0.25 * (((a00 + a10) + a01) + a11) : (T)0.5 * (a00 + a10);
                    const T add = rodd ? od : ev;
                    u[i][e] = unk ? u[i][e] + add : u[i][e];
                }
            }
        };
        if (gy0 & 1) correct(std::integral_constant<int, 1>{});
        else correct(std::integral_constant<int, 0>{});
    }

    MGX_PHASE_AFTER(b[RW - 1][W - 1]);
    MGX_PHASE_AFTER(u[RW - 1][W - 1]);

    int buf = 0;
    auto halo_rows = [&](const T (&a)[RW][W], T (&up)[W], T (&dn)[W]) {
        edge[buf][wv][0][lane] = vmake(a[0]);
        edge[buf][wv][1][lane] = vmake(a[RW - 1]);
        __syncthreads();
        const V uv = wv > 0 ? edge[buf][wv - 1][1][lane] : vzero((V*)nullptr);
        const V dv = wv < NW - 1 ? edge[buf][wv + 1][0][lane] : vzero((V*)nullptr);
#pragma unroll
        for (int e = 0; e < W; ++e) { up[e] = vget(uv, e); dn[e] = vget(dv, e); }
        buf ^= 1;
    };
    for (int j = 1; j <= levels; ++j) {
        T up[W], dn[W];
        halo_rows(u, up, dn);
        const int colour = (j - 1) & 1;
        T prev[W];
// ... 229 lines not shown
```

### multigrid_nikhil_c-_amd/csrc/mgx_launch.hpp

```cpp
#pragma once

#include "../../include/mgx.h"
#include "mgx_kernels.hpp"
#include "mgx_pass_plan.hpp"

#include <algorithm>

namespace mgx {

inline long level_pitch(int level, int dtype)
{
    const long N = 1L << level;
    const long align = (dtype == MGX_DTYPE_F64) ? 32 : 64;
    return (N + 1 + align - 1) / align * align;
}

template <typename T> struct JacobiCoef { T c0, c1; };
template <typename T>
JacobiCoef<T> jacobi_coef(double omega)
{
    const T om = (T)omega;
    return {(T)(1.0 - (double)om), (T)((double)om / 4.0)};
}

template <typename T_, int SM_, int AR_> struct KernelSet { using T = T_; static constexpr int SM = SM_, AR = AR_; };
template <typename F>
decltype(auto) with_kernel_set(bool f64, int smoother, int arith, F&& f)
{
    const bool rbgs = (smoother == MGX_SMOOTHER_RBGS);
    if (f64) return rbgs ? f(KernelSet<double, 1, 0>{}) : (arith ? f(KernelSet<double, 0, 1>{}) : f(KernelSet<double, 0, 0>{}));
    return rbgs ? f(KernelSet<float, 1, 0>{}) : (arith ? f(KernelSet<float, 0, 1>{}) : f(KernelSet<float, 0, 0>{}));
}

template <typename T>
int launch_jacobi(const T* vin, const T* b, T* vout, int N, long pitch, int row_lo, int row_hi,
                  double omega, int rpc, hipStream_t st, int rows_alloc, int arith = 0)
{
    if (row_hi <= row_lo) return MGX_OK;
    if (row_lo < 1 || row_hi > rows_alloc - 1) return MGX_ERR_INVALID;
    const auto [c0, c1] = jacobi_coef<T>(omega);
    if (rpc <= 0) {
        const Launch g = make_launch(N, VecOf<T>::W, row_hi - row_lo, 1);
        if (arith) hipLaunchKernelGGL((k_jacobi_rows<T, 1>), dim3(g.blocks), dim3(kBlock), 0, st, vin, b, vout, N, pitch,
                                      row_lo, row_hi, g.strips, c0, c1, rows_alloc);
        else hipLaunchKernelGGL((k_jacobi_rows<T, 0>), dim3(g.blocks), dim3(kBlock), 0, st, vin, b, vout, N, pitch,
                                row_lo, row_hi, g.strips, c0, c1, rows_alloc);
        return MGX_OK;
    }
    const Launch g = make_launch(N, VecOf<T>::W, row_hi - row_lo, rpc);
    if (arith) hipLaunchKernelGGL((k_jacobi<T, 1>), dim3(g.blocks), dim3(kBlock), 0, st, vin, b, vout, N, pitch,
                                  row_lo, row_hi, g.R, g.strips, g.chunks, c0, c1, rows_alloc);
    else hipLaunchKernelGGL((k_jacobi<T, 0>), dim3(g.blocks), dim3(kBlock), 0, st, vin, b, vout, N, pitch,
                            row_lo, row_hi, g.R, g.strips, g.chunks, c0, c1, rows_alloc);
    return MGX_OK;
}

template <typename T>
void launch_rbgs(const T* vin, const T* b, T* vout, int N, long pitch, int row_lo, int row_hi,
                 int row_parity, int bnd_lo, int bnd_hi, int rpc, hipStream_t st)
{
    if (row_hi <= row_lo) return;
    const Launch g = make_launch(N, VecOf<T>::W, row_hi - row_lo, rpc);
    hipLaunchKernelGGL((k_rbgs<T>), dim3(g.blocks), dim3(kBlock), 0, st, vin, b, vout, N, pitch,
                       row_lo, row_hi, g.R, g.strips, g.chunks, row_parity, bnd_lo, bnd_hi);
}

template <typename T, int K, int SM, int AR>
void launch_fused_k(const T* vin, const T* b, T* vout, int N, long pitch, int row_lo, int row_hi,
                    T c0, T c1, int bnd_lo, int bnd_hi, int row_parity, int R, hipStream_t st, int rows_alloc, int zero_in)
{
    constexpr int OUT = fused_out_lanes<K, VecOf<T>::W>();
    R = trip_rows(R, 2 * K, trip_steps<T>(), 1);
    Launch g = make_launch(N, VecOf<T>::W, row_hi - row_lo, R);
    g.strips = (N / VecOf<T>::W + OUT - 1) / OUT;
    const long waves = (long)g.strips * g.chunks;
    g.blocks = (int)(((waves + kWavesPerBlock - 1) / kWavesPerBlock + 7) / 8 * 8);
    hipLaunchKernelGGL((k_jacobi_fused<T, K, SM, AR>), dim3(g.blocks), dim3(kBlock), 0, st, vin, b, vout, N, pitch,
                       row_lo, row_hi, g.R, g.strips, g.chunks, c0, c1, bnd_lo, bnd_hi, row_parity, rows_alloc, zero_in);
}

template <typename T, int SM, int AR>
bool launch_fused(int K, const T* vin, const T* b, T* vout, int N, long pitch, int row_lo, int row_hi,
                  T c0, T c1, int bnd_lo, int bnd_hi, int row_parity, int R, hipStream_t st, int rows_alloc, int zero_in)
{
    switch (K) {
        case 2: launch_fused_k<T, 2, SM, AR>(vin, b, vout, N, pitch, row_lo, row_hi, c0, c1, bnd_lo, bnd_hi, row_parity, R, st, rows_alloc, zero_in); return true;
        case 4: launch_fused_k<T, 4, SM, AR>(vin, b, vout, N, pitch, row_lo, row_hi, c0, c1, bnd_lo, bnd_hi, row_parity, R, st, rows_alloc, zero_in); return true;
        case 6: launch_fused_k<T, 6, SM, AR>(vin, b, vout, N, pitch, row_lo, row_hi, c0, c1, bnd_lo, bnd_hi, row_parity, R, st, rows_alloc, zero_in); return true;
        case 8: launch_fused_k<T, 8, SM, AR>(vin, b, vout, N, pitch, row_lo, row_hi, c0, c1, bnd_lo, bnd_hi, row_parity, R, st, rows_alloc, zero_in); return true;
        case 10: launch_fused_k<T, 10, SM, AR>(vin, b, vout, N, pitch, row_lo, row_hi, c0, c1, bnd_lo, bnd_hi, row_parity, R, st, rows_alloc, zero_in); return true;
        default: break;
    }
    if constexpr (SM == 0) {
        switch (K) {
            case 3: launch_fused_k<T, 3, 0, AR>(vin, b, vout, N, pitch, row_lo, row_hi, c0, c1, bnd_lo, bnd_hi, row_parity, R, st, rows_alloc, zero_in); return true;
            case 5: launch_fused_k<T, 5, 0, AR>(vin, b, vout, N, pitch, row_lo, row_hi, c0, c1, bnd_lo, bnd_hi, row_parity, R, st, rows_alloc, zero_in); return true;
            default: break;
        }
    }
    return false;
}

struct FoldArgs {
    const void* coarse_e = nullptr;
    void* coarse_b = nullptr;
    void* coarse_zero = nullptr;
    int restrict_mode = 0;
    double* partial = nullptr;
    long cpitch = 0;
    int zero_in = 0;
    int row_lo = 0, row_hi = 0;
    CycleWin win{0, 0, 0, 0, 0, 0};
};

inline GeomKnobs geom_knobs()
{
    GeomKnobs k;
    k.edge_short = env_int("MGX_EDGE_SHORT", 1) != 0;
    k.edge_pct = env_int("MGX_EDGE_PCT", 23);
    k.last_pct = env_int("MGX_LAST_PCT", 38);
    k.min_chunk = std::max(8, env_int("MGX_MIN_CHUNK", 16));
    k.min_rounds = std::max(1, env_int("MGX_MIN_ROUNDS", 1));
    k.min_rounds_rows = env_int("MGX_MIN_ROUNDS_ROWS", 1024);
    k.pair = env_int("MGX_PAIR", 1) != 0;
    k.pair_ratio = std::max(100, env_int("MGX_PAIR_RATIO", 130));
    k.pair_max_rows = env_int("MGX_PAIR_MAX_ROWS", 640);
    k.pair_min_rows = env_int("MGX_PAIR_MIN_ROWS", 150);
    return k;
}
template <typename T, int K, int PRE, int POST, int SM, int AR>
int launch_cycle_k(const T* vin, const T* b, T* vout, const FoldArgs& fa, int N, long pitch, T c0, T c1, int R,
                   hipStream_t st)
{
    constexpr int OUT = cycle_out_lanes<K, POST, VecOf<T>::W>();
    constexpr bool BL = cycle_b_in_lds<T, K, POST, SM>();
    constexpr int E = (POST == 1 ? 3 : (POST == 2 ? 2 : 0)) + (cycle_skew<T, K, PRE, POST, SM, AR>() > 0 ? 1 : 0);
    constexpr int kTripSteps = BL ? kBRing : trip_steps<T>();
    const int row_lo = fa.row_lo, row_hi = fa.row_hi;
    const CycleWin& win = fa.win;
    if (POST == 1 && !(row_lo & 1)) return -1;
    const int strips = (N / VecOf<T>::W + OUT - 1) / OUT;
    const bool auto_rows = R < 0;
    if (auto_rows) R = -R;
    constexpr int ETOP = POST ? 1 : 0, EBOT = POST == 1 ? 2 : (POST == 2 ? 1 : 0);
    const bool top_edge = (row_lo - K - ETOP) < std::max(win.row_first, 1) || (PRE && ((row_lo - K - ETOP) >> 1) < win.crow_first);
    const bool bot_edge = (row_hi + K + EBOT - 1) > std::min(win.row_last, N - 1) || (PRE && ((row_hi + K + EBOT) >> 1) > win.crow_last);
    GeomKnobs kn = BL ? geom_knobs() : GeomKnobs();
    if (sizeof(T) == 4 && BL) kn.pair_min_rows = std::min(kn.pair_min_rows, env_int("MGX_PAIR_MIN_ROWS_F32", 100));
    const CycleGeom g = cycle_geom_pick(row_lo, row_hi, strips, 2 * K + E, kTripSteps, R, auto_rows, BL, kn, top_edge, bot_edge);
    const int blocks = g.blocks;
    const T w = (fa.restrict_mode == MGX_RESTRICT_FW16) ? (T)0.0625 : (T)0.25;
    hipLaunchKernelGGL((k_jacobi_cycle<T, K, PRE, POST, SM, AR>), dim3(blocks), dim3(kBlock), 0, st, vin, b, vout,
                       (const T*)fa.coarse_e, (T*)fa.coarse_b, (T*)fa.coarse_zero, w, fa.partial, N, pitch, fa.cpitch,
                       row_lo, row_hi, g.R, strips, g.chunks, g.Re, g.chunks_e, g.row_last0, g.Rl, g.RB, g.n_tall, g.n_short, g.Rf, c0, c1, fa.zero_in, win);
    return blocks;
}

template <typename T, int PRE, int POST, int SM, int AR>
int launch_cycle(int K, const T* vin, const T* b, T* vout, const FoldArgs& fa, int N, long pitch, T c0, T c1, int R,
                 hipStream_t st)
{
    switch (K) {
        case 2: return launch_cycle_k<T, 2, PRE, POST, SM, AR>(vin, b, vout, fa, N, pitch, c0, c1, R, st);
        case 4: return launch_cycle_k<T, 4, PRE, POST, SM, AR>(vin, b, vout, fa, N, pitch, c0, c1, R, st);
        case 6: return launch_cycle_k<T, 6, PRE, POST, SM, AR>(vin, b, vout, fa, N, pitch, c0, c1, R, st);
        default: break;
    }
    if constexpr (sizeof(T) == 8 || PRE == 1 || POST == 0) {
        if (K == 8) return launch_cycle_k<T, 8, PRE, POST, SM, AR>(vin, b, vout, fa, N, pitch, c0, c1, R, st);
    }
    if constexpr (!(PRE == 1 && POST == 1) && !(SM == 1 && POST == 1) && !(sizeof(T) == 4 && PRE == 1 && POST == 2) &&
                  !(sizeof(T) == 4 && POST == 1 && AR == 0)) {
        if (K == 10) return launch_cycle_k<T, 10, PRE, POST, SM, AR>(vin, b, vout, fa, N, pitch, c0, c1, R, st);
    }
    if constexpr (SM == 0) {
        switch (K) {
            case 1: return launch_cycle_k<T, 1, PRE, POST, 0, AR>(vin, b, vout, fa, N, pitch, c0, c1, R, st);
            case 3: return launch_cycle_k<T, 3, PRE, POST, 0, AR>(vin, b, vout, fa, N, pitch, c0, c1, R, st);
            case 5: return launch_cycle_k<T, 5, PRE, POST, 0, AR>(vin, b, vout, fa, N, pitch, c0, c1, R, st);
            default: break;
        }
    }
    return -1;
}

template <int PRE_, int POST_> struct Stages { static constexpr int PRE = PRE_, POST = POST_; };
template <typename F>
int with_stages(bool pre, int post, F&& f)
{
    if (pre) return post == 2 ? f(Stages<1, 2>{}) : (post == 1 ? f(Stages<1, 1>{}) : f(Stages<1, 0>{}));
    return post == 2 ? f(Stages<0, 2>{}) : (post == 1 ? f(Stages<0, 1>{}) : f(Stages<0, 0>{}));
}

template <typename T, int SM, int PRE, int POST, int AR>
int launch_tile(const T* vin, const T* b, T* vout, const FoldArgs& fa, int N, long pitch, T c0, T c1, int levels,
                hipStream_t st)
{
    const int He = levels + tile_extra<POST>();
    const int TH = kTileSY - 2 * He, TW = kTileSX - 2 * He;
    if (TH < 8 || TW < 8) return -1;
    const int row_lo = fa.row_lo, row_hi = fa.row_hi;
    const CycleWin& win = fa.win;
    const int tiles_y = (row_hi - row_lo + TH - 1) / TH, tiles_x = (N - 1 + TW - 1) / TW;
    if (tiles_y < 1) return 0;
    const T w = (fa.restrict_mode == MGX_RESTRICT_FW16) ? (T)0.0625 : (T)0.25;
    hipLaunchKernelGGL((k_tile_smooth<T, SM, PRE, POST, AR>), dim3(tiles_y * tiles_x), dim3(kBlock), 0, st, vin, b, vout,
                       (const T*)fa.coarse_e, (T*)fa.coarse_b, (T*)fa.coarse_zero, w, fa.partial, N, pitch, fa.cpitch,
                       levels, c0, c1, tiles_x, fa.zero_in, row_lo, row_hi, win);
    return tiles_y * tiles_x;
}

template <typename T, int SM, int PRE, int POST, int AR>
int launch_tile_wide(const T* vin, const T* b, T* vout, const FoldArgs& fa, int N, long pitch, T c0, T c1, int levels,
                     int rw, hipStream_t st)
{
    if (VecOf<T>::W == 4) rw = 8;
    const int row_lo = fa.row_lo, row_hi = fa.row_hi;
    const CycleWin& win = fa.win;
    const TileWideGeom g = tile_wide_geom(N, row_lo, row_hi, levels + tile_extra<POST>(), VecOf<T>::W, rw);
    if (g.TH < 8 || g.TW < 8) return -1;
    if (g.tiles_y < 1) return 0;
    const T w = (fa.restrict_mode == MGX_RESTRICT_FW16) ? (T)0.0625 : (T)0.25;
    const dim3 grid(g.tiles_y * g.tiles_x), block(kTileWideWaves * kWave);
    if (rw == 8)
        hipLaunchKernelGGL((k_tile_wide<T, SM, PRE, POST, AR, 8>), grid, block, 0, st, vin, b, vout, (const T*)fa.coarse_e,
                           (T*)fa.coarse_b, (T*)fa.coarse_zero, w, fa.partial, N, pitch, fa.cpitch, levels, c0, c1, g.tiles_x,
                           fa.zero_in, row_lo, row_hi, win);
    else if constexpr (VecOf<T>::W == 2) {
        if (rw != 10) return -1;
        hipLaunchKernelGGL((k_tile_wide<T, SM, PRE, POST, AR, 10>), grid, block, 0, st, vin, b, vout, (const T*)fa.coarse_e,
                           (T*)fa.coarse_b, (T*)fa.coarse_zero, w, fa.partial, N, pitch, fa.cpitch, levels, c0, c1, g.tiles_x,
                           fa.zero_in, row_lo, row_hi, win);
    } else {
        return -1;
    }
    return g.tiles_y * g.tiles_x;
}

template <typename T, int SM, int AR>
int launch_tile_pass(const T* vin, const T* b, T* vout, const FoldArgs& fa, int N, long pitch, T c0, T c1, int levels,
                     int band, bool pre, int post, hipStream_t st)
{
    return with_stages(pre, post, [&](auto s) {
        using S = decltype(s);
        return band ? launch_tile_wide<T, SM, S::PRE, S::POST, AR>(vin, b, vout, fa, N, pitch, c0, c1, levels, band, st)
                    : launch_tile<T, SM, S::PRE, S::POST, AR>(vin, b, vout, fa, N, pitch, c0, c1, levels, st);
    });
}

template <typename T>
void launch_restrict(const T* v, const T* b, T* cb, T* czero, int N, long pitch, long cpitch,
                     int crow_lo, int crow_hi, int fine_row_off, int mode, bool fused, int rpc, hipStream_t st)
{
    if (crow_hi <= crow_lo) return;
    Launch g = make_launch(N, VecOf<T>::W, crow_hi - crow_lo, rpc > 0 ? (rpc + 1) / 2 : 0);
    const T w = (mode == MGX_RESTRICT_FW16) ? (T)0.0625 : (T)0.25;
    if (fused)
        hipLaunchKernelGGL((k_restrict<T, true>), dim3(g.blocks), dim3(kBlock), 0, st, v, b, cb, czero, N, pitch,
                           cpitch, crow_lo, crow_hi, fine_row_off, g.R, g.strips, g.chunks, w);
    else
        hipLaunchKernelGGL((k_restrict<T, false>), dim3(g.blocks), dim3(kBlock), 0, st, v, b, cb, czero, N, pitch,
                           cpitch, crow_lo, crow_hi, fine_row_off, g.R, g.strips, g.chunks, w);
}

template <typename T>
void launch_prolong(T* v, const T* e, int N, long pitch, long cpitch, int row_lo, int row_hi,
                    int fine_row_off, bool add, int rpc, hipStream_t st)
{
    if (row_hi <= row_lo) return;
    const Launch g = make_launch(N, VecOf<T>::W, row_hi - row_lo, rpc);
    if (add)
        hipLaunchKernelGGL((k_prolong<T, true>), dim3(g.blocks), dim3(kBlock), 0, st, v, e, N, pitch, cpitch,
                           row_lo, row_hi, fine_row_off, g.R, g.strips, g.chunks);
    else
        hipLaunchKernelGGL((k_prolong<T, false>), dim3(g.blocks), dim3(kBlock), 0, st, v, e, N, pitch, cpitch,
                           row_lo, row_hi, fine_row_off, g.R, g.strips, g.chunks);
}

template <typename T> long sumsq_blocks(int N, int rows, int rpc)
{
    return make_launch(N, VecOf<T>::W, rows, rpc).blocks;
}

template <typename T, int MODE>
void launch_residual(const T* v, const T* b, void* out, long pitch_out, double* partial, double* sum_dev,
                     double inv_scale, int N, long pitch, int row_lo, int row_hi, int rpc, hipStream_t st,
                     long partial_cap, int rows_alloc)
{
    Launch g = make_launch(N, VecOf<T>::W, row_hi - row_lo, rpc);
    if (MODE != 0 && partial_cap >= 0 && g.blocks > partial_cap) {
        const int R = (int)(((long)g.strips * (row_hi - row_lo) / kWavesPerBlock + partial_cap - 9) / (partial_cap - 8)) + 1;
        g = make_launch(N, VecOf<T>::W, row_hi - row_lo, R);
    }
    hipLaunchKernelGGL((k_residual<T, MODE>), dim3(g.blocks), dim3(kBlock), 0, st, v, b, out, pitch_out, partial,
                       inv_scale, N, pitch, row_lo, row_hi, g.R, g.strips, g.chunks, rows_alloc);
    if (MODE != 0)
        hipLaunchKernelGGL(k_reduce_partials, dim3(1), dim3(kReduceThreads), 0, st, partial, g.blocks, sum_dev);
}


#define MGX_FOR_SMAR(X, T) X(T, 0, 0) X(T, 0, 1) X(T, 1, 0)
#define MGX_DECL_CYCLE_PP(T, PRE, POST, SM, AR) \
    extern template int launch_cycle<T, PRE, POST, SM, AR>(int, const T*, const T*, T*, const FoldArgs&, int, long, T, T, int, hipStream_t);
#define MGX_DECL_CYCLE(T, SM, AR) MGX_DECL_CYCLE_PP(T, 1, 2, SM, AR) MGX_DECL_CYCLE_PP(T, 1, 0, SM, AR) MGX_DECL_CYCLE_PP(T, 0, 1, SM, AR) \
    MGX_DECL_CYCLE_PP(T, 0, 2, SM, AR) MGX_DECL_CYCLE_PP(T, 1, 1, SM, AR)
#define MGX_DECL_FUSED(T, SM, AR) \
    extern template bool launch_fused<T, SM, AR>(int, const T*, const T*, T*, int, long, int, int, T, T, int, int, int, int, hipStream_t, int, int);
#define MGX_DECL_TILE(T, SM, AR) \
    extern template int launch_tile_pass<T, SM, AR>(const T*, const T*, T*, const FoldArgs&, int, long, T, T, int, int, bool, int, hipStream_t);
#if !defined(MGX_INST_KIND) && !defined(MGX_SINGLE_TU)
MGX_FOR_SMAR(MGX_DECL_CYCLE, double) MGX_FOR_SMAR(MGX_DECL_CYCLE, float)
MGX_FOR_SMAR(MGX_DECL_FUSED, double) MGX_FOR_SMAR(MGX_DECL_FUSED, float)
MGX_FOR_SMAR(MGX_DECL_TILE, double) MGX_FOR_SMAR(MGX_DECL_TILE, float)
#endif

}
```

### multigrid_nikhil_c-_amd/csrc/mgx_pass_plan.hpp

```cpp
#pragma once

#include "../../include/mgx.h"
#include "mgx_geom.hpp"

#include <algorithm>
#include <cstdlib>
#include <vector>

namespace mgx {

inline int env_int(const char* name, int dflt)
{
    const char* s = getenv(name);
    return (s && *s) ? atoi(s) : dflt;
}

struct FuseCfg {
    int kmax; int rows; int min_n; int fold_kmax; int fold_kmax_big; int tile_max_n; int tile_k; int fold_kmax_nopost;
    int tile_wide; int tile_short_n;
    int plan_pre[8] = {0}; int n_pre = 0; int plan_post[8] = {0}; int n_post = 0; int plan_min_n = 8192;
    int arith = 0;
};

inline int fuse_rows_deep(int N, int rows)
{
    const int strips = (N / 2 + 51) / 52;
    const int cpr = std::max(1, 2048 / strips);
    for (int m = 1; m <= 64; ++m) {
        const int R = (rows + m * cpr - 1) / (m * cpr);
        if (R <= 200) return std::max(R, 16);
    }
    return 64;
}

inline bool fuse_rows_auto(const FuseCfg& fc, int N, int K, bool f64)
{
    return fc.rows <= 0 && K >= (f64 ? 8 : 10) && N >= 2048;
}

inline int shallow_big_n() { static const int n = env_int("MGX_SHALLOW_BIG_N", 8192); return n; }
inline int shallow_mid_rows() { static const int r = env_int("MGX_SHALLOW_ROWS_MID", 48); return r; }

inline int fuse_rows(const FuseCfg& fc, int N, int K, bool f64 = true, int rows = 0)
{
    if (fc.rows > 0) return fc.rows;
    if (K <= 2) {
        static const int big2 = env_int("MGX_SHALLOW2_ROWS_BIG", 96);
        return N >= shallow_big_n() ? big2 : (N >= 4096 ? shallow_mid_rows() : 8);
    }
    if (K <= 4) {
        static const int big = env_int("MGX_SHALLOW_ROWS_BIG", 96);
        return N >= shallow_big_n() ? big : (N >= 4096 ? shallow_mid_rows() : 16);
    }
    if (f64 && K >= 8 && N >= 2048) return fuse_rows_deep(N, rows > 0 ? rows : N - 1);
    int R = N / 128;
    if (R < 8) R = 8;
    if (R > (f64 ? 64 : 32)) R = f64 ? 64 : 32;
    return R;
}

inline FuseCfg fuse_cfg()
{
    FuseCfg f;
    f.kmax = env_int("MGX_FUSE", 10);
    if (f.kmax < 1) f.kmax = 1;
    if (f.kmax > 10) f.kmax = 10;
    f.rows = env_int("MGX_FUSE_ROWS", 0);
    if (f.rows < 0) f.rows = 0;
    f.min_n = std::max(64, env_int("MGX_FUSE_MIN_N", 256));
    f.fold_kmax = std::max(1, std::min(f.kmax, env_int("MGX_FOLD_KMAX", 10)));
    f.fold_kmax_big = std::max(1, std::min(f.kmax, env_int("MGX_FOLD_KMAX_BIG", 10)));
    f.tile_wide = std::max(0, std::min(2, env_int("MGX_TILE_WIDE", 1)));
    f.tile_short_n = env_int("MGX_TILE_SHORT_N", 512);
    f.tile_max_n = std::max(0, env_int("MGX_TILE_MAX_N", 1024));
    f.tile_k = std::max(2, std::min(10, env_int("MGX_TILE_K", 10)));
    f.fold_kmax_nopost = std::max(1, std::min(f.kmax, env_int("MGX_FOLD_KMAX_NOPOST", 10)));
    auto parse = [](const char* name, int* out) {
        const char* v = std::getenv(name);
        int n = 0;
        while (v && *v && n < 8) {
            char* end = nullptr;
            const long k = std::strtol(v, &end, 10);
            if (end == v || k < 1 || k > 10) return 0;
            out[n++] = (int)k;
            v = (*end == ',') ? end + 1 : end;
            if (*end && *end != ',') return 0;
        }
        return n;
    };
    f.n_pre = parse("MGX_PLAN_PRE", f.plan_pre);
    f.n_post = parse("MGX_PLAN_POST", f.plan_post);
    f.plan_min_n = env_int("MGX_PLAN_MIN_N", 8192);
    return f;
}

inline bool cycle_k_supported(int K, bool rbgs, bool f64, int post, bool pre, int arith)
{
    if (K == 10) return !(pre && post == 1) && !(rbgs && post == 1) && !(!f64 && pre && post == 2) && !(!f64 && post == 1 && arith == 0);
    if (K == 8 && !f64 && !pre && post != 0) return false;
    return rbgs ? (K == 2 || K == 4 || K == 6 || K == 8) : (K >= 1 && K <= 8 && K != 7);
}

inline bool fused_k_supported(int K, bool rbgs)
{
    return K == 2 || K == 4 || K == 6 || K == 8 || K == 10 || (!rbgs && (K == 3 || K == 5));
}

inline int tile_band(const FuseCfg& fc, int N, bool f64)
{
    return (fc.tile_wide >= (f64 ? 1 : 2)) ? tile_wide_rw(N, fc.tile_short_n) : 0;
}

constexpr double kFuseRate64[11] = {0, 1.00, 1.80, 2.45, 3.16, 3.81, 4.80, 0, 5.60, 0, 5.63};
constexpr double kFuseRate32[11] = {0, 1.00, 1.67, 2.38, 3.10, 3.77, 4.26, 0, 4.98, 0, 4.67};
constexpr double kFuseRateGS64[11] = {0, 1.00, 1.81, 2.50, 3.19, 3.12, 0, 0, 0, 0, 0};
constexpr double kFuseRateGS32[11] = {0, 1.00, 1.79, 2.20, 2.87, 2.69, 0, 0, 0, 0, 0};

inline double fold_pass_cost(int K, bool rbgs, int post, bool f64, int arith)
{
    if (!cycle_k_supported(K, rbgs, f64, post, false, arith)) return -1.0;
    if (rbgs) return K <= 4 ? 1.0 : (K == 6 ? 1.1 : (K == 8 ? 1.3 : 2.4));
    if (K <= 5) return 1.0;
    if (!f64) return K == 6 ? 1.34 : (K == 8 ? 1.53 : 1.75);
    if (K == 6) return 1.05;
    if (K == 8) return 1.12;
    return 1.46;
}

template <typename Cost>
std::vector<int> split_sweeps(int mu, int smax, double launch, double eps, Cost cost)
{
    std::vector<double> best(mu + 1, 1e300);
    std::vector<int> pick(mu + 1, 1);
    best[0] = 0.0;
    for (int m = 1; m <= mu; ++m)
        for (int k = 1; k <= std::min(m, smax); ++k) {
            const double c = cost(k, m);
            if (c < 0.0) continue;
            const double t = best[m - k] + c + launch;
            if (t < best[m] - eps) { best[m] = t; pick[m] = k; }
        }
    std::vector<int> parts;
    for (int m = mu; m > 0; m -= pick[m]) parts.push_back(pick[m]);
    return parts;
}

enum PassKind {
    PASS_JACOBI,
    PASS_RBGS,
    PASS_FUSED,
    PASS_FOLDED,
    PASS_TILE,
};

struct Pass {
    int kind;
    int K;
    bool pre; int post;
    bool zero_in;
    int lo, hi;
    int R;
};

struct BlockReq {
    int smoother = MGX_SMOOTHER_JACOBI; bool f64 = true;
    int N = 0, row0 = 0, rows = 0;
    int row_lo = 0, row_hi = 0;
    int mu = 0;
    bool pre = false;
    int post = 0;
    bool zero_in = false;
    bool widen = true;
    bool strict = false;
    long tile_points = 0;
    int rpc = 0;
};

inline bool fold_plan(const FuseCfg& fc, const BlockReq& q, std::vector<Pass>* plan)
{
    plan->clear();
    const bool rbgs = (q.smoother == MGX_SMOOTHER_RBGS);
    const int per = rbgs ? 2 : 1, N = q.N, mu = q.mu;
    const int first = 1 - q.row0, last = N - q.row0;
    {
        const int lo = std::max(std::max(q.row_lo, first), 1), hi = std::min(std::min(q.row_hi, last), q.rows - 1);
        const bool whole = q.row_lo <= first && q.row_hi >= last;
        if (fc.tile_max_n > 0 && hi > lo && (long)(hi - lo) * N <= q.tile_points && (per * mu <= fc.tile_k || whole)) {
            const int smax = std::max(1, fc.tile_k / per), np = (mu + smax - 1) / smax;
            for (int p = 0; p < np; ++p) {
                const int sw = mu / np + (p < mu % np ? 1 : 0);
                plan->push_back({PASS_TILE, per * sw, q.pre && p == 0, p == np - 1 ? q.post : 0, q.zero_in && p == 0,
                                 lo + q.row0, hi + q.row0, tile_band(fc, N, q.f64)});
            }
            return true;
        }
    }
    const bool staged = q.pre || q.post != 0;
    const bool fuse = fc.kmax > per && N >= fc.min_n && (q.row_hi - q.row_lo) >= 64 && mu <= 64;
    std::vector<int> parts;
    if (!staged) {
        const double* rate = rbgs ? (q.f64 ? kFuseRateGS64 : kFuseRateGS32) : (q.f64 ? kFuseRate64 : kFuseRate32);
        if (fuse)
            parts = split_sweeps(mu, std::max(1, std::min(fc.kmax, 10) / per), 0.02, 0.0,
                                 [&](int k, int) { return rate[k] > 0.0 ? (double)k / rate[k] : -1.0; });
        else
            parts.assign(std::max(mu, 0), 1);
    } else {
        const int* forced = nullptr;
        int nf = 0;
        if (!q.pre && q.post == 1) { forced = fc.plan_pre; nf = fc.n_pre; }
        else if (q.pre) { forced = fc.plan_post; nf = fc.n_post; }
        if (nf > 0 && N >= fc.plan_min_n) {
            int sum = 0;
            bool ok = true;
            for (int i = 0; i < nf; ++i) {
                sum += forced[i];
                const int K = per * forced[i];
                const bool folded = (i == 0 && q.pre) || (i == nf - 1 && q.post != 0);
                const int Q = (i == nf - 1) ? q.post : 0;
                ok = ok && K <= 10 && (folded ? cycle_k_supported(K, rbgs, q.f64, Q, q.pre && i == 0, fc.arith) : (K != 7 && K != 9 && (!rbgs || K % 2 == 0)));
            }
            if (ok && sum == mu) parts.assign(forced, forced + nf);
        }
        if (parts.empty()) {
            int kcap = N >= 8192 ? fc.fold_kmax_big : fc.fold_kmax;
            if (q.post == 0) kcap = std::min(kcap, fc.fold_kmax_nopost);
            if (rbgs) kcap = std::min(kcap, env_int("MGX_FOLD_KMAX_GS", 10));
            if (q.pre && q.post == 1) kcap = std::min(kcap, 8);
            parts = split_sweeps(mu, std::max(1, kcap / per), 1e-3, 1e-12, [&](int k, int m) {
                if (k == mu && m == mu && !cycle_k_supported(per * k, rbgs, q.f64, q.post, q.pre, fc.arith)) return -1.0;
                return fold_pass_cost(per * k, rbgs, q.post, q.f64, fc.arith);
            });
            std::sort(parts.begin(), parts.end(), [](int a, int b) { return a > b; });
        }
    }
    const int np = (int)parts.size();
    const int stage_rows = q.post == 2 ? 1 : (q.post == 1 ? 2 : 0);
    int done = 0;
    for (int p = 0; p < np; ++p) {
        const int sw = parts[p], K = per * sw;
        const bool P = q.pre && p == 0, zin = q.zero_in && p == 0;
        const int Q = (p == np - 1) ? q.post : 0;
        const int ext = q.widen ? per * (mu - (done + sw)) + (p != np - 1 ? stage_rows : 0) : 0;
        int lo = std::max(q.row_lo - ext, first), hi = std::min(q.row_hi + ext, last);
        if (q.strict && hi > lo && (std::max(lo - K, first - 1) < 0 || std::min(hi + K - 1, last) > q.rows - 1)) return false;
        lo = std::max(lo, 1);
        hi = std::min(hi, q.rows - 1);
        const int kind = (P || Q) ? PASS_FOLDED : (!rbgs && K == 1) ? PASS_JACOBI : (rbgs && !staged && !fuse) ? PASS_RBGS : PASS_FUSED;
        int R = q.rpc;
        if (kind == PASS_FUSED || kind == PASS_FOLDED) R = fuse_rows(fc, N, K, q.f64, hi - lo);
        if (hi > lo) {
            if (kind == PASS_FOLDED) {
                if (!cycle_k_supported(K, rbgs, q.f64, Q, P, fc.arith)) return false;
                if (Q == 1 && !((lo + q.row0) & 1)) return false;
                if (fuse_rows_auto(fc, N, K, q.f64)) R = -R;
            }
            if (kind == PASS_FUSED && !fused_k_supported(K, rbgs)) return false;
            if (zin && (kind == PASS_JACOBI || kind == PASS_RBGS)) return false;
        }
        plan->push_back({kind, K, P, Q, zin, lo + q.row0, hi + q.row0, R});
        done += sw;
    }
    return true;
}

}
```

Baseline: 1150 billion.

## Add seam-paired waves that march toward each other to share chunk halos

Introduces a seam mode for the deep K=10 f64 temporal-blocked Jacobi cycle kernel. Pairs of waves in the same block process adjacent row chunks in opposite directions: one marches down and one marches up through mirrored row indexing. At the start they exchange intermediate level rows through LDS with barriers, which is meant to avoid recomputing the K-row halo on both sides of a chunk boundary. It adds a new tile-to-block mapping and a geometry picker, costs extra LDS ring slots and barrier syncs, and by default is enabled only for POST==1 passes with at most 48 rows per chunk.

```diff
diff --git a/multigrid_nikhil_c-_amd/csrc/mgx.hip b/multigrid_nikhil_c-_amd/csrc/mgx.hip
--- a/multigrid_nikhil_c-_amd/csrc/mgx.hip
+++ b/multigrid_nikhil_c-_amd/csrc/mgx.hip
@@ -696,6 +696,7 @@
     FoldArgs fa;
     fa.restrict_mode = restrict_mode;
     fa.partial = partial;
+    fa.seam = fc.seam;
     fa.win.row_first = std::max(row0, 0);
     fa.win.row_last = std::min(row0 + q.rows - 1, N);
     fa.win.crow_first = 0; fa.win.crow_last = -1; fa.win.emit_lo = 0; fa.win.emit_hi = 0;
diff --git a/multigrid_nikhil_c-_amd/csrc/mgx_geom.hpp b/multigrid_nikhil_c-_amd/csrc/mgx_geom.hpp
--- a/multigrid_nikhil_c-_amd/csrc/mgx_geom.hpp
+++ b/multigrid_nikhil_c-_amd/csrc/mgx_geom.hpp
@@ -251,6 +251,140 @@
     return g;
 }
 
+struct STile { int strip, r0, r1; bool active; int dir; };
+
+struct SeamCounts {
+    int nt, ns;
+    int ntp, nsp;
+    int wt, ws;
+    int pt, ps;
+    int n_edge;
+};
+
+MGX_GEOM_HD SeamCounts seam_counts(int strips, int chunks, int chunks_e, int n_tall, int n_short)
+{
+    const int si = strips - 2;
+    SeamCounts c;
+    c.nt = n_tall > 0 ? n_tall : chunks - 3;
+    c.ns = n_tall > 0 ? n_short : 0;
+    c.ntp = (c.nt >> 1) * si; c.nsp = (c.ns >> 1) * si;
+    c.wt = c.ntp >> 1; c.ws = c.nsp >> 1;
+    c.pt = 2 * (c.ntp & 1) + (c.nt & 1) * si; c.ps = 2 * (c.nsp & 1) + (c.ns & 1) * si;
+    c.n_edge = 3 * si + 2 * chunks_e;
+    return c;
+}
+
+MGX_GEOM_HD STile seam_tile_at(int block, int wave, int strips, int chunks, int chunks_e, int R, int Re, int row_lo, int row_hi,
+                               int row_last0, int Rl, int RB, int n_tall, int n_short, int Rf)
+{
+    const int si = strips - 2;
+    const int xcd = block & 7;
+    const int nth = block >> 3;
+    const SeamCounts c = seam_counts(strips, chunks, chunks_e, n_tall, n_short);
+    STile t;
+    t.strip = 0; t.r0 = 0; t.r1 = 0; t.active = false; t.dir = 0;
+    const bool second = n_tall > 0 && nth >= kGeomCusPerXcd;
+    const int n = second ? nth - kGeomCusPerXcd : nth;
+    const int plain_n = second ? c.ps : c.n_edge + c.pt;
+    const int seam_w = second ? c.ws : c.wt;
+    const int np = second ? c.nsp : c.ntp;
+    const int nc = second ? c.ns : c.nt;
+    const int h = second ? RB : R;
+    const int base = row_lo + Rf + (second ? c.nt * R : 0);
+    const int pp = (plain_n + 7) >> 3, pw = (pp + kGeomWavesPerBlock - 1) / kGeomWavesPerBlock, sw = (seam_w + 7) >> 3;
+    int chunk = -1;
+    if (n < pw) {
+        const int lw = n * kGeomWavesPerBlock + wave;
+        int k = xcd * pp + lw;
+        if (lw < pp && k < plain_n) {
+            if (!second && k < c.n_edge) {
+                t.active = true;
+                if (k < 3 * si) {
+                    const int which = k / si;
+                    t.strip = 1 + (k - which * si);
+                    t.r0 = which == 0 ? row_lo : (which == 1 ? row_last0 : row_last0 + Rl);
+                    t.r1 = which == 0 ? row_lo + Rf : (which == 1 ? row_last0 + Rl : row_hi);
+                } else {
+                    const int e = k - 3 * si;
+                    t.strip = (e & 1) ? strips - 1 : 0;
+                    t.r0 = row_lo + (e >> 1) * Re;
+                    t.r1 = geom_min(t.r0 + Re, row_hi);
+                }
+                t.active = t.r0 < t.r1;
+                return t;
+            }
+            if (!second) k -= c.n_edge;
+            const int odd_pair = 2 * (np & 1);
+            if (k < odd_pair) { const int p = np - 1; chunk = 2 * (p / si) + k; t.strip = 1 + p % si; }
+            else { chunk = nc - 1; t.strip = 1 + (k - odd_pair); }
+        }
+    } else if (n - pw < sw) {
+        const int w = xcd * sw + (n - pw);
+        if (w < seam_w) {
+            const int p = 2 * w + (wave >> 1);
+            chunk = 2 * (p / si) + ((wave & 1) ? 0 : 1);
+            t.strip = 1 + p % si;
+            t.dir = (wave & 1) ? -1 : 1;
+        }
+    }
+    if (chunk >= 0) {
+        t.r0 = base + chunk * h;
+        t.r1 = geom_min(t.r0 + h, row_last0);
+        t.active = t.r0 < t.r1;
+    }
+    return t;
+}
+
+inline int seam_blocks(const CycleGeom& g, int strips)
+{
+    const SeamCounts c = seam_counts(strips, g.chunks, g.chunks_e, g.n_tall, g.n_short);
+    auto wgs = [](int plain_n, int seam_w) { return (((plain_n + 7) / 8) + kGeomWavesPerBlock - 1) / kGeomWavesPerBlock + (seam_w + 7) / 8; };
+    const int first = wgs(c.n_edge + c.pt, c.wt);
+    if (g.n_tall == 0) return 8 * first;
+    if (first > kGeomCusPerXcd) return -1;
+    return 8 * (kGeomCusPerXcd + wgs(c.ps, c.ws));
+}
+
+inline bool seam_geom_pick(int row_lo, int row_hi, int strips, int extra_plain, int extra_seam, int trip, int R, bool auto_rows,
+                           const GeomKnobs& kn, bool top_edge, bool bot_edge, CycleGeom* out, bool paired_too = true)
+{
+    if (strips < 4 || !(row_lo & 1)) return false;
+    const CycleGeom plain = cycle_geom_pick(row_lo, row_hi, strips, extra_plain, trip, R, auto_rows, true, kn, top_edge, bot_edge);
+    const int rounds = (plain.blocks + kGeomResidentBlocks - 1) / kGeomResidentBlocks;
+    CycleGeom g = cycle_geom_pick(row_lo, row_hi, strips, extra_seam, trip, R, auto_rows, true, kn, top_edge, bot_edge);
+    if (g.n_tall > 0 && !paired_too) return false;
+    if (g.row_last0 != 0 && g.n_tall > 0) {
+        const int mid = g.row_last0 - (row_lo + g.Rf);
+        int best_nt = g.n_tall, best_ns = g.n_short, best_odd = (g.n_tall & 1) + (g.n_short & 1);
+        for (int nt = g.n_tall - 1; nt <= g.n_tall + 1 && best_odd > 0; nt += 2) {
+            if (nt < 1 || (long)nt * g.R > mid - g.RB) continue;
+            const int ns = (mid - nt * g.R + g.RB - 1) / g.RB;
+            CycleGeom c = g;
+            c.n_tall = nt; c.n_short = ns; c.chunks = 3 + nt + ns;
+            const int b = seam_blocks(c, strips);
+            if (b < 0 || b > rounds * kGeomResidentBlocks) continue;
+            if ((nt & 1) + (ns & 1) < best_odd) { best_odd = (nt & 1) + (ns & 1); best_nt = nt; best_ns = ns; }
+        }
+        g.n_tall = best_nt; g.n_short = best_ns; g.chunks = 3 + best_nt + best_ns;
+        g.waves = (long)g.chunks * (strips - 2) + 2L * g.chunks_e;
+    }
+    for (int more = 0; more < 6; ++more) {
+        if (g.row_last0 == 0) return false;
+        if ((g.R & 1) || (g.Rf & 1) || (g.n_tall > 0 && (g.RB & 1))) return false;
+        const SeamCounts c = seam_counts(strips, g.chunks, g.chunks_e, g.n_tall, g.n_short);
+        if (c.wt + c.ws < 1) return false;
+        const int blocks = seam_blocks(g, strips);
+        if (blocks >= 0 && blocks <= rounds * kGeomResidentBlocks) {
+            g.blocks = blocks;
+            *out = g;
+            return true;
+        }
+        if (!auto_rows || g.n_tall > 0) return false;
+        g = cycle_geom_pick(row_lo, row_hi, strips, extra_seam, trip, g.R + trip, false, true, kn, top_edge, bot_edge);
+    }
+    return false;
+}
+
 constexpr int kTileWideWaves = 8;
 
 struct TileWideGeom {
diff --git a/multigrid_nikhil_c-_amd/csrc/mgx_kernels.hpp b/multigrid_nikhil_c-_amd/csrc/mgx_kernels.hpp
--- a/multigrid_nikhil_c-_amd/csrc/mgx_kernels.hpp
+++ b/multigrid_nikhil_c-_amd/csrc/mgx_kernels.hpp
@@ -836,7 +836,7 @@
 template <int K, int POST, int W> constexpr int cycle_out_lanes() { return kWave - 2 * ((cycle_halo_cols<K, POST>() + W - 1) / W); }
 
 template <typename T, int CW> struct CycleState {
-    T ct[CW], tc[CW], em[CW], mc[CW];
+    T ct[CW], tc[CW], em[CW], mc[CW], sb[CW];
     T ea[CW + 1];
     double acc;
 };
@@ -851,6 +851,8 @@
     long cpitch; int NC;
     int r0, r1, y_end;
     bool zero_in;
+    bool first;
+    int mir;
     CycleWin win;
 };
 
@@ -899,14 +901,21 @@
     }
 }
 
-template <typename T, bool EDGE, bool ZIN = false>
+template <typename T, bool EDGE, bool ZIN = false, int DIR = 1>
 __device__ __forceinline__ void
 cycle_loads(typename VecOf<T>::type& in, typename VecOf<T>::type& bn, int y,
             const T* __restrict__ pv, const T* __restrict__ pb, long pitch, int N, int y_end, bool ld, bool zero_in,
-            const CycleWin& win, const FastOut& fo)
+            const CycleWin& win, const FastOut& fo, int mir = 0)
 {
     using V = typename VecOf<T>::type;
-    if constexpr (!EDGE) {
+    static_assert(DIR > 0 || !EDGE, "only interior bodies march up");
+    if constexpr (DIR < 0) {
+        const int ya = mir - y;
+        const int yi = max(min(ya, win.row_last), win.row_first), yb = max(min(ya + 1, win.row_last), win.row_first);
+        if constexpr (ZIN) in = vzero((V*)nullptr);
+        else in = bload_s((V*)nullptr, fo.in, fo.lane_off, (unsigned)(yi - fo.rb) * fo.pitch_bytes);
+        bn = bload_s((V*)nullptr, fo.rhs, fo.lane_off, (unsigned)(yb - fo.rb) * fo.pitch_bytes);
+    } else if constexpr (!EDGE) {
         const int yi = min(y, win.row_last), yb = max(min(y - 1, win.row_last), win.row_first);
         if constexpr (ZIN) in = vzero((V*)nullptr);
         else in = bload_s((V*)nullptr, fo.in, fo.lane_off, (unsigned)(yi - fo.rb) * fo.pitch_bytes);
@@ -981,6 +990,15 @@
     if (POST == 2 && AR == 0 && K == 10) return false;
     return cycle_b_in_lds<T, K, POST, SM>() && SM == 0 && POST != 0 && K > kRawLds && cycle_skew<T, K, PRE, POST, SM, AR>() == 0;
 }
+template <typename T, int K, int PRE, int POST, int SM, int AR> constexpr bool cycle_seam()
+{
+    constexpr bool variant = (PRE == 1 && POST == 0) || (PRE == 0 && POST == 1);
+    return sizeof(T) == 8 && K == 10 && variant && SM == 0 && cycle_b_in_lds<T, K, POST, SM>() &&
+           cycle_skew<T, K, PRE, POST, SM, AR>() == 0 && K + 1 < kBRing;
+}
+constexpr int kSeamSlots = 2 * kBRing + 4;
+__device__ __forceinline__ void seam_sync() { asm volatile("s_waitcnt lgkmcnt(0)\n\ts_barrier" ::: "memory"); }
+
 #ifndef MGX_PFD_DEEP
 #define MGX_PFD_DEEP 0
 #endif
@@ -992,10 +1010,11 @@
 constexpr int kPrefetchMax = MGX_PFD_DEEP > kPrefetch ? MGX_PFD_DEEP : kPrefetch;
 template <typename T, bool BL, bool EDGE, int POST> constexpr int cycle_cpfd() { return (BL && !(EDGE && POST == 0)) ? cycle_pfd<BL, POST, EDGE>() : 1; }
 
-template <typename T, int K, int PRE, int POST, int SM, bool EDGE, int RP, bool BL, bool ZIN, int AR, int YP>
+template <typename T, int K, int PRE, int POST, int SM, bool EDGE, int RP, bool BL, bool ZIN, int AR, int YP, int DIR = 1, int SS = -1>
 __device__ __forceinline__ void
 cycle_step(typename VecOf<T>::type (&lev)[K + 1][3], typename VecOf<T>::type (&bw)[BL ? 1 : K + 1], lds_vec_ptr<T> ring,
-           lds_vec_ptr<T> ring2, typename VecOf<T>::type (&rawq)[cycle_rawq<T, K, PRE, POST, SM, AR>() ? kBRing : 1],
+           lds_vec_ptr<T> ring2,
+           typename VecOf<T>::type (&rawq)[cycle_rawq<T, K, PRE, POST, SM, AR>() ? kBRing : 1],
            typename VecOf<T>::type (&nin)[kPfStages], typename VecOf<T>::type (&nbn)[kPfStages], PreFetch<T, VecOf<T>::W / 2>& pe,
            CycleState<T, VecOf<T>::W / 2>& cs, int y,
            const T* __restrict__ pv, const T* __restrict__ pb, T* __restrict__ po,
@@ -1011,15 +1030,46 @@
     constexpr int bnd_lo = 0;
     const int bnd_hi = N;
     const int r0 = ca.r0, r1 = ca.r1;
+    constexpr int RSO = DIR < 0 ? kBRing + 4 : 0;
+    constexpr int SX_MINE = kBRing + (DIR < 0 ? 2 : 0), SX_OTHER = kBRing + (DIR < 0 ? 0 : 2);
+    constexpr int SX_LAST = POST ? K : K - 1;
 
     if constexpr (EDGE) __builtin_amdgcn_sched_barrier(0);
     V in = nin[0];
     const V bn = nbn[0];
 #pragma unroll
     for (int q = 0; q + 1 < kPfStages; ++q) { nin[q] = nin[q + 1]; nbn[q] = nbn[q + 1]; }
-    cycle_loads<T, EDGE, ZIN>(nin[kPfStages - 1], nbn[kPfStages - 1], y + cycle_pfd<BL, POST, EDGE>(), pv, pb, pitch, N, ca.y_end, ld, ca.zero_in, ca.win, fo);
+    cycle_loads<T, EDGE, ZIN, DIR>(nin[kPfStages - 1], nbn[kPfStages - 1], y + cycle_pfd<BL, POST, EDGE>(), pv, pb, pitch, N, ca.y_end, ld, ca.zero_in, ca.win, fo, ca.mir);
     const ColMask cm = col_mask(col, N);
-    if (PRE) {
+    if constexpr (PRE != 0 && DIR < 0) {
+        static_assert(YP >= 0 && !EDGE, "the up-march knows its row parity");
+        constexpr int YA = 1 - YP;
+        constexpr int CPFD = cycle_cpfd<T, BL, EDGE, POST>();
+        const int ya = ca.mir - y;
+        T o[W], nw[CW + 1];
+        if constexpr (YA == 1) {
+#pragma unroll
+            for (int k = 0; k <= CW; ++k) nw[k] = pe.b[k];
+        }
+        if constexpr (((YA + CPFD) & 1) == 1) coarse_row<T, EDGE>(pe.b, (ya - CPFD) >> 1, cld, ca.win, fo);
+#pragma unroll
+        for (int k = 0; k < CW; ++k) {
+            if constexpr (YA == 0) {
+                o[2 * k] = cs.ea[k];
+                o[2 * k + 1] = (T)0.5 * (cs.ea[k] + cs.ea[k + 1]);
+            } else {
+                const T ab = nw[k] + cs.ea[k];
+                o[2 * k] = (T)0.5 * ab;
+                o[2 * k + 1] = (T)0.25 * ((ab + nw[k + 1]) + cs.ea[k + 1]);
+            }
+        }
+        if constexpr (YA == 1) {
+#pragma unroll
+            for (int k = 0; k <= CW; ++k) cs.ea[k] = nw[k];
+        }
+        if constexpr (W == 2) { in.x = in.x + o[0]; in.y = in.y + o[1]; }
+        else { in.x = in.x + o[0]; in.y = in.y + o[1]; in.z = in.z + o[2]; in.w = in.w + o[3]; }
+    } else if (PRE) {
         T o[W];
         bool row_zero = false;
         if constexpr (YP < 0) {
@@ -1079,7 +1129,7 @@
     else b0 = bn;
     if constexpr (BL) {
         asm volatile("" : "+v"(ring));
-        ring_put(ring, ring_slot(RP), b0);
+        ring_put(ring, RSO + ring_slot(RP), b0);
         if constexpr (RAWQ) {
             asm volatile("" : "+v"(ring2));
             rawq[ring_slot(RP)] = ring_get(ring2, RP % kRawLds);
@@ -1103,14 +1153,20 @@
     };
     V dying = lev[SK][S_NEW];
     lev[0][S_NEW] = in;
+    if constexpr (SS == 0) { if (ca.first) ring_put(ring, SX_MINE, in); }
+    if constexpr (SS >= 1 && SS - 1 <= SX_LAST) if (ca.first) {
+        static_assert(cycle_skew<T, K, PRE, POST, SM, AR>() == 0 && !EDGE, "seam waves run the serial chain of an interior body");
+        seam_sync();
+        lev[SS - 1][S_OLD] = ring_get(ring, SX_OTHER + ((SS - 1) & 1));
+    }
     auto level = [&](auto jc, auto bc) {
         constexpr int j = decltype(jc)::value;
         constexpr bool inB = decltype(bc)::value;
         const int row = y - j - (inB ? 1 : 0);
         const V cb = bwin(std::integral_constant<int, j - 1 + (inB ? 1 : 0)>{});
-        const V& lo = (inB && j == SK + 1) ? dying : lev[j - 1][S_OLD];
+        const V& lo = DIR < 0 ? lev[j - 1][S_NEW] : ((inB && j == SK + 1) ? dying : lev[j - 1][S_OLD]);
         const V& mi = (inB && j == SK + 1) ? lev[j - 1][S_OLD] : lev[j - 1][S_MID];
-        const V& hi = (inB && j == SK + 1) ? lev[j - 1][S_MID] : lev[j - 1][S_NEW];
+        const V& hi = DIR < 0 ? lev[j - 1][S_OLD] : ((inB && j == SK + 1) ? lev[j - 1][S_MID] : lev[j - 1][S_NEW]);
         V o;
         if constexpr (PREMUL) o = jacobi_vec_pre<AR>(lo, mi, hi, cb, c0, c1);
         else o = level_op<T, SM, AR>(j, lo, mi, hi, cb, c0, c1, row + (int)(col & 1));
@@ -1119,22 +1175,23 @@
             mask_sel(o, cm, !(rw > bnd_lo && rw < bnd_hi));
         }
         if constexpr (j == K) {
-            const unsigned at = (unsigned)(row - fo.rb) * fo.pitch_bytes + fo.lane_off;
+            const unsigned at = (unsigned)((DIR < 0 ? ca.mir - row : row) - fo.rb) * fo.pitch_bytes + fo.lane_off;
             bstore(o, fo.out, (st && row >= r0 && row < r1) ? at : kOobOffset);
         }
         if (j < K || POST) lev[j][S_NEW] = o;
+        if constexpr (SS >= 1 && j == SS && j <= SX_LAST) { if (ca.first) ring_put(ring, SX_MINE + (SS & 1), o); }
     };
     if constexpr (SK == 0) {
         if constexpr (BL) {
             static_for<1, (kRingAhead < MLAST ? kRingAhead : MLAST) + 1>([&](auto mc) {
                 constexpr int m = decltype(mc)::value;
-                rq[m] = ring_get(ring, ring_slot(RP - m));
+                rq[m] = ring_get(ring, RSO + ring_slot(RP - m));
             });
         }
         static_for<1, K + 1>([&](auto jc) {
             constexpr int j = decltype(jc)::value;
             if constexpr (BL && j + kRingAhead <= MLAST) {
-                rq[j + kRingAhead] = ring_get(ring, ring_slot(RP - (j + kRingAhead)));
+                rq[j + kRingAhead] = ring_get(ring, RSO + ring_slot(RP - (j + kRingAhead)));
                 __builtin_amdgcn_sched_barrier(0);
             }
             level(jc, std::false_type{});
@@ -1158,7 +1215,8 @@
         V rawb;
         if constexpr (RAWQ) rawb = rawq[ring_slot(RP - (K - kRawLds))];
         else rawb = bwin(std::integral_constant<int, K + SKD>{});
-        V res = residual_vec(lev[K][S_OLD], lev[K][S_MID], lev[K][S_NEW], rawb);
+        V res = DIR < 0 ? residual_vec(lev[K][S_NEW], lev[K][S_MID], lev[K][S_OLD], rawb)
+                        : residual_vec(lev[K][S_OLD], lev[K][S_MID], lev[K][S_NEW], rawb);
         if constexpr (EDGE) {
             const int rw = opaque_s(rho);
             mask_sel(res, cm, !(rw > bnd_lo && rw < bnd_hi));
@@ -1174,6 +1232,40 @@
             const T l = from_left(last(res));
             if constexpr (W == 2) { cl[0] = l; cc[0] = res.x; cr[0] = res.y; }
             else { cl[0] = l; cc[0] = res.x; cr[0] = res.y; cl[1] = res.y; cc[1] = res.z; cr[1] = res.w; }
+            if constexpr (DIR < 0) {
+                static_assert(YP >= 0 && SKD == 0 && !EDGE, "the up-march knows its row parity");
+                constexpr int RA = 1 - ((YP + K + 1) & 1);
+                if constexpr (RA == 1) {
+                    const int J = (ca.mir - rho + 1) >> 1;
+                    T o[CW];
+#pragma unroll
+                    for (int k = 0; k < CW; ++k) {
+                        T corners = (cl[k] + cr[k]) + cs.ct[k]; corners = corners + cs.tc[k];
+                        const T edges = (cs.em[k] + cc[k]) + cs.sb[k];
+                        o[k] = wgt * ((corners + (T)2 * edges) + (T)4 * cs.mc[k]);
+                    }
+                    const bool emit = rho > r0 && rho <= r1 && J >= ca.win.emit_lo && J < ca.win.emit_hi;
+                    const unsigned at = (st && emit) ? ((unsigned)(J - fo.crb) * fo.cpitch_bytes + fo.clane_off) : kOobOffset;
+                    if constexpr (CW == 1) { bstore8(o[0], fo.cb, at); bstore8((T)0, fo.cz, at); }
+                    else { bstore8(make_float2((float)o[0], (float)o[1]), fo.cb, at); bstore8(make_float2(0.f, 0.f), fo.cz, at); }
+#pragma unroll
+                    for (int k = 0; k < CW; ++k) { cs.ct[k] = cl[k]; cs.tc[k] = cr[k]; cs.sb[k] = cc[k]; }
+                } else {
+#pragma unroll
+                    for (int k = 0; k < CW; ++k) { cs.em[k] = cl[k] + cr[k]; cs.mc[k] = cc[k]; }
+                }
+                if constexpr (SS == K + 1) if (ca.first) {
+                    seam_sync();
+                    const V pr = ring_get(ring, SX_OTHER + 1);
+                    const T pl = from_left(last(pr));
+                    if constexpr (W == 2) { cs.ct[0] = pl; cs.sb[0] = pr.x; cs.tc[0] = pr.y; }
+                    else { cs.ct[0] = pl; cs.sb[0] = pr.x; cs.tc[0] = pr.y; cs.ct[1] = pr.y; cs.sb[1] = pr.z; cs.tc[1] = pr.w; }
+                }
+            } else {
+            if constexpr (SS == K + 1) if (ca.first) {
+                ring_put(ring, SX_MINE + 1, res);
+                seam_sync();
+            }
             constexpr int RHOP = YP < 0 ? -1 : ((YP + K + 1 + SKD) & 1);
             const int I = (rho - 1) >> 1;
             if constexpr (RHOP < 0) {
@@ -1222,23 +1314,27 @@
 #pragma unroll
                 for (int k = 0; k < CW; ++k) { cs.em[k] = (cl[k] + cr[k]) + cs.tc[k]; cs.mc[k] = cc[k]; }
             }
-        }
-    }
-}
-
-template <typename T, int K, int PRE, int POST, int SM, bool EDGE, bool ZIN, int AR>
+            }
+        }
+    }
+}
+
+template <typename T, int K, int PRE, int POST, int SM, bool EDGE, bool ZIN, int AR, int SEAM = 0>
 __device__ __forceinline__ double
 cycle_body(const T* __restrict__ pv, const T* __restrict__ pb, T* __restrict__ po,
            const T* __restrict__ coarse_e, T* __restrict__ coarse_b, T* __restrict__ coarse_zero, T wgt,
            long pitch, long cpitch, long col, int N, int r0, int r1, bool ld, bool st, T c0, T c1, bool zero_in,
-           const CycleWin& win, lds_vec_ptr<T> ring, lds_vec_ptr<T> ring2, const FastOut& fo)
-{
+           const CycleWin& win, lds_vec_ptr<T> ring, lds_vec_ptr<T> ring2, const FastOut& fo,
+           int mir = 0)
+{
+    constexpr int DIR = SEAM < 0 ? -1 : 1;
+    static_assert(SEAM == 0 || (cycle_seam<T, K, PRE, POST, SM, AR>() && !EDGE), "seam waves: interior bodies of the seam variants");
     constexpr bool BL = cycle_b_in_lds<T, K, POST, SM>();
     constexpr bool RAWQ = cycle_rawq<T, K, PRE, POST, SM, AR>();
     using V = typename VecOf<T>::type;
     constexpr int W = VecOf<T>::W;
     constexpr int CW = W / 2;
-    constexpr int EBOT = POST == 1 ? 2 : (POST == 2 ? 1 : 0);
+    constexpr int EBOT = SEAM < 0 ? (POST ? 1 : 0) : (POST == 1 ? 2 : (POST == 2 ? 1 : 0));
     const V Z = vzero((V*)nullptr);
     const long ccol = col / 2;
     const bool cld = ld && (ccol + CW < cpitch);
@@ -1250,7 +1346,7 @@
     for (int j = 0; j < (BL ? 1 : K + 1); ++j) bw[j] = Z;
     if constexpr (BL) {
 #pragma unroll
-        for (int q = 0; q < kBRing; ++q) ring_put(ring, q, Z);
+        for (int q = 0; q < kBRing; ++q) ring_put(ring, (DIR < 0 ? kBRing + 4 : 0) + q, Z);
     }
     V rawq[RAWQ ? kBRing : 1];
 #pragma unroll
@@ -1262,13 +1358,13 @@
     CycleState<T, CW> cs;
     cs.acc = 0.0;
 #pragma unroll
-    for (int k = 0; k < CW; ++k) cs.ct[k] = cs.tc[k] = cs.em[k] = cs.mc[k] = (T)0;
+    for (int k = 0; k < CW; ++k) cs.ct[k] = cs.tc[k] = cs.em[k] = cs.mc[k] = cs.sb[k] = (T)0;
 #pragma unroll
     for (int k = 0; k <= CW; ++k) cs.ea[k] = (T)0;
     CycleArgs ca;
-    ca.cpitch = cpitch; ca.NC = N / 2; ca.r0 = r0; ca.r1 = r1; ca.zero_in = zero_in; ca.win = win;
-    constexpr int PAR = cycle_par<T, K, POST, SM>();
-    const int y0 = cycle_y0<T, K, POST, SM>(r0);
+    ca.cpitch = cpitch; ca.NC = N / 2; ca.r0 = r0; ca.r1 = r1; ca.zero_in = zero_in; ca.win = win; ca.mir = mir; ca.first = false;
+    constexpr int PAR = SEAM ? 1 : cycle_par<T, K, POST, SM>();
+    const int y0 = SEAM ? r0 : cycle_y0<T, K, POST, SM>(r0);
     ca.y_end = r1 + K + EBOT + (cycle_skew<T, K, PRE, POST, SM, AR>() > 0 ? 1 : 0);
     constexpr int kRound = BL ? kBRing : trip_steps<T>();
     const int steps = (ca.y_end - y0 + kRound - 1) / kRound * kRound;
@@ -1283,8 +1379,13 @@
     }
 #pragma unroll
     for (int q = 0; q < PFD; ++q)
-        cycle_loads<T, EDGE, ZIN>(nin[q][0], nbn[q][0], y0 + q, pv, pb, pitch, N, ca.y_end, ld, ca.zero_in, ca.win, fo);
-    if (PRE) {
+        cycle_loads<T, EDGE, ZIN, DIR>(nin[q][0], nbn[q][0], y0 + q, pv, pb, pitch, N, ca.y_end, ld, ca.zero_in, ca.win, fo, mir);
+    if constexpr (PRE != 0 && DIR < 0) {
+        coarse_row<T, EDGE>(cs.ea, (mir - y0) >> 1, cld, ca.win, fo);
+#pragma unroll
+        for (int q = 0; q < CPFD; ++q)
+            if (((PAR + q) & 1) == 0) coarse_row<T, EDGE>(pe[q].b, (mir - (y0 + q)) >> 1, cld, ca.win, fo);
+    } else if (PRE) {
         if constexpr (PAR < 0) {
 #pragma unroll
             for (int q = 0; q < CPFD; ++q) coarse_loads<T, EDGE>(pe[q], y0 + q, coarse_e, cpitch, ccol, N, cld, ca.win, fo);
@@ -1295,7 +1396,7 @@
                 if (((PAR + q) & 1) == 1) coarse_row<T, EDGE>(pe[q].b, ((y0 + q) >> 1) + 1, cld, ca.win, fo);
         }
     }
-#define MGX_CSTEP(RP, Y) cycle_step<T, K, PRE, POST, SM, EDGE, RP, BL, ZIN, AR, (PAR < 0 ? -1 : ((PAR + (RP)) & 1))>(lev, bw, ring, ring2, rawq, nin[(RP) % PFD], nbn[(RP) % PFD], pe[(RP) % CPFD], cs, Y, pv, pb, po, coarse_e, coarse_b, coarse_zero, wgt, pitch, col, ccol, N, ca, ld, cld, st, c0, c1, fo)
+#define MGX_CSTEP(RP, Y) cycle_step<T, K, PRE, POST, SM, EDGE, RP, BL, ZIN, AR, (PAR < 0 ? -1 : ((PAR + (RP)) & 1)), DIR, -1>(lev, bw, ring, ring2, rawq, nin[(RP) % PFD], nbn[(RP) % PFD], pe[(RP) % CPFD], cs, Y, pv, pb, po, coarse_e, coarse_b, coarse_zero, wgt, pitch, col, ccol, N, ca, ld, cld, st, c0, c1, fo)
     if constexpr (BL) {
 #define MGX_CTRIP(Y) do { MGX_CSTEP(0, Y); MGX_CSTEP(1, Y + 1); MGX_CSTEP(2, Y + 2); MGX_CSTEP(3, Y + 3); MGX_CSTEP(4, Y + 4); \
                           MGX_CSTEP(5, Y + 5); MGX_CSTEP(6, Y + 6); MGX_CSTEP(7, Y + 7); MGX_CSTEP(8, Y + 8); MGX_CSTEP(9, Y + 9); \
@@ -1311,7 +1412,17 @@
         }
         __builtin_amdgcn_s_setprio(0);
 #else
-        for (int y = y0; y < y0 + steps; y += kBRing) MGX_CTRIP(y);
+        if constexpr (SEAM != 0) {
+#define MGX_SSTEP(RP, Y) cycle_step<T, K, PRE, POST, SM, EDGE, RP, BL, ZIN, AR, ((PAR + (RP)) & 1), DIR, RP>(lev, bw, ring, ring2, rawq, nin[(RP) % PFD], nbn[(RP) % PFD], pe[(RP) % CPFD], cs, Y, pv, pb, po, coarse_e, coarse_b, coarse_zero, wgt, pitch, col, ccol, N, ca, ld, cld, st, c0, c1, fo)
+            for (int y = y0; y < y0 + steps; y += kBRing) {
+                ca.first = (y == y0);
+                MGX_SSTEP(0, y); MGX_SSTEP(1, y + 1); MGX_SSTEP(2, y + 2); MGX_SSTEP(3, y + 3); MGX_SSTEP(4, y + 4); MGX_SSTEP(5, y + 5);
+                MGX_SSTEP(6, y + 6); MGX_SSTEP(7, y + 7); MGX_SSTEP(8, y + 8); MGX_SSTEP(9, y + 9); MGX_SSTEP(10, y + 10); MGX_SSTEP(11, y + 11);
+            }
+#undef MGX_SSTEP
+        } else {
+            for (int y = y0; y < y0 + steps; y += kBRing) MGX_CTRIP(y);
+        }
 #endif
 #undef MGX_CTRIP
     } else if constexpr (trip_steps<T>() == 12) {
@@ -1341,7 +1452,8 @@
                T* __restrict__ coarse_b, T* __restrict__ coarse_zero, T wgt,
                double* __restrict__ partial,
                int N, long pitch, long cpitch, int row_lo, int row_hi, int R, int strips, int chunks, int Re, int chunks_e,
-               int row_last0, int Rl, int RB, int n_tall, int n_short, int Rf, T c0, T c1, int zero_in, CycleWin win)
+               int row_last0, int Rl, int RB, int n_tall, int n_short, int Rf, T c0, T c1, int zero_in, CycleWin win,
+               int seam)
 {
     constexpr int W = VecOf<T>::W;
     constexpr int XC = cycle_halo_cols<K, POST>();
@@ -1351,10 +1463,44 @@
     constexpr int EBOT = POST == 1 ? 2 : (POST == 2 ? 1 : 0);
     __shared__ double wsum[kWavesPerBlock];
     constexpr bool BL = cycle_b_in_lds<T, K, POST, SM>();
-    __shared__ typename LdsVec<T>::v bring[BL ? kWavesPerBlock * kBRing * kWave : 1];
+    constexpr bool SEAMK = cycle_seam<T, K, PRE, POST, SM, AR>();
+    constexpr int kRingRows = SEAMK ? kSeamSlots / 2 : kBRing;
+    __shared__ typename LdsVec<T>::v bring[BL ? kWavesPerBlock * kRingRows * kWave : 1];
     constexpr bool RAWQ = cycle_rawq<T, K, PRE, POST, SM, AR>();
     __shared__ typename LdsVec<T>::v braw[RAWQ ? kWavesPerBlock * kRawLds * kWave : 1];
-    const CTile t = cycle_tile(strips, chunks, chunks_e, R, Re, row_lo, row_hi, row_last0, Rl, RB, n_tall, n_short, Rf);
+    CTile t;
+    int sdir = 0;
+    if (SEAMK && seam) {
+        auto seam_ok = [&](const STile& s) -> bool {
+            if (!s.active || s.dir == 0) return false;
+            const int x0 = s.strip * OUT - HL;
+            bool ok = (x0 >= 1) && ((long)(x0 + kWave + 1) * W < N) && !(PRE != 0 && zero_in);
+            if (s.dir > 0) {
+                const int y1 = s.r1 + K + EBOT - 1;
+                ok = ok && (s.r0 & 1) && (s.r0 - 1 >= win.row_first) && (s.r0 > 1) && (y1 < N) && (y1 <= win.row_last);
+                if (PRE) ok = ok && (s.r0 >> 1) >= win.crow_first && ((y1 + 1) >> 1) <= win.crow_last;
+            } else {
+                const int y0u = s.r0 - K - ETOP;
+                ok = ok && (s.r1 & 1) && (y0u > 0) && (y0u >= win.row_first) && (s.r1 < N) && (s.r1 <= win.row_last);
+                if (PRE) ok = ok && (y0u >> 1) >= win.crow_first && (s.r1 >> 1) <= win.crow_last;
+            }
+            return ok;
+        };
+        const int wave = __builtin_amdgcn_readfirstlane(threadIdx.x >> 6);
+        bool all = true;
+        STile mine;
+        mine.strip = 0; mine.r0 = 0; mine.r1 = 0; mine.active = false; mine.dir = 0;
+#pragma unroll
+        for (int w = 0; w < kWavesPerBlock; ++w) {
+            const STile s = seam_tile_at((int)blockIdx.x, w, strips, chunks, chunks_e, R, Re, row_lo, row_hi, row_last0, Rl, RB, n_tall, n_short, Rf);
+            all = all && seam_ok(s);
+            if (w == wave) mine = s;
+        }
+        t.strip = mine.strip; t.r0 = mine.r0; t.r1 = mine.r1; t.active = mine.active;
+        sdir = all ? mine.dir : 0;
+    } else {
+        t = cycle_tile(strips, chunks, chunks_e, R, Re, row_lo, row_hi, row_last0, Rl, RB, n_tall, n_short, Rf);
+    }
     double acc = 0.0;
 #ifdef MGX_WAVE_TRACE
     const long long trace_t0 = wall_clock64();
@@ -1362,7 +1508,7 @@
     if (t.active) {
         const int lane = threadIdx.x & 63;
         const int wv = __builtin_amdgcn_readfirstlane(threadIdx.x >> 6);
-        lds_vec_ptr<T> ring = (lds_vec_ptr<T>)&bring[BL ? (wv * kBRing * kWave + lane) : 0];
+        lds_vec_ptr<T> ring = (lds_vec_ptr<T>)&bring[BL ? ((sdir != 0 ? (wv & ~1) : wv) * kRingRows * kWave + lane) : 0];
         lds_vec_ptr<T> ring2 = (lds_vec_ptr<T>)&braw[RAWQ ? (wv * kRawLds * kWave + lane) : 0];
         const int vx0 = t.strip * OUT - HL;
         const int vx = vx0 + lane;
@@ -1371,7 +1517,7 @@
         const bool st = (lane >= HL) && (lane < kWave - HL) && (vx < N / W);
         const int r0 = t.r0, r1 = t.r1;
         constexpr int kRound = BL ? kBRing : trip_steps<T>();
-        const int y_first = cycle_y0<T, K, POST, SM>(r0) - 1;
+        const int y_first = sdir == 0 ? cycle_y0<T, K, POST, SM>(r0) - 1 : (sdir > 0 ? r0 - 1 : r0 - K - kBRing - kPrefetchMax - 2);
         constexpr int SKD = cycle_skew<T, K, PRE, POST, SM, AR>() > 0 ? 1 : 0;
         const int y_lastp = (r0 - K - ETOP) + ((r1 + K + EBOT + SKD) - (r0 - K - ETOP) + kRound - 1) / kRound * kRound + kPrefetchMax;
         const int y0c = r0 - K - ETOP, y1c = r1 + K + EBOT - 1;
@@ -1396,7 +1542,26 @@
         fo.cz = make_rsrc((POST == 1 && coarse_zero) ? coarse_zero + c_at : nullptr, (POST == 1 && coarse_zero) ? c_bytes : 0u);
         fo.lane_off = (unsigned)(col * (long)sizeof(T));
         fo.clane_off = (unsigned)((col / 2) * (long)sizeof(T));
-        if (interior) {
+        if constexpr (SEAMK) {
+            if (sdir != 0) interior = false;
+        }
+        if (SEAMK && sdir != 0) {
+            if constexpr (SEAMK) {
+                const bool zin = PRE == 0 && zero_in;
+                if (sdir > 0 && zin)
+                    acc = cycle_body<T, K, PRE, POST, SM, false, PRE == 0, AR, 1>(vin + col, rhs + col, vout + col, coarse_e, coarse_b, coarse_zero, wgt,
+                                                                              pitch, cpitch, col, N, r0, r1, true, st, c0, c1, true, win, ring, ring2, fo, 0);
+                else if (sdir > 0)
+                    acc = cycle_body<T, K, PRE, POST, SM, false, false, AR, 1>(vin + col, rhs + col, vout + col, coarse_e, coarse_b, coarse_zero, wgt,
+                                                                           pitch, cpitch, col, N, r0, r1, true, st, c0, c1, false, win, ring, ring2, fo, 0);
+                else if (zin)
+                    acc = cycle_body<T, K, PRE, POST, SM, false, PRE == 0, AR, -1>(vin + col, rhs + col, vout + col, coarse_e, coarse_b, coarse_zero, wgt,
+                                                                               pitch, cpitch, col, N, r1, r1 + (r1 - r0), true, st, c0, c1, true, win, ring, ring2, fo, 2 * r1 - 1);
+                else
+                    acc = cycle_body<T, K, PRE, POST, SM, false, false, AR, -1>(vin + col, rhs + col, vout + col, coarse_e, coarse_b, coarse_zero, wgt,
+                                                                            pitch, cpitch, col, N, r1, r1 + (r1 - r0), true, st, c0, c1, false, win, ring, ring2, fo, 2 * r1 - 1);
+            }
+        } else if (interior) {
             if (PRE == 0 && zero_in)
                 acc = cycle_body<T, K, PRE, POST, SM, false, PRE == 0, AR>(vin + col, rhs + col, vout + col, coarse_e, coarse_b, coarse_zero, wgt,
                                                                       pitch, cpitch, col, N, r0, r1, true, st, c0, c1, true, win, ring, ring2, fo);
diff --git a/multigrid_nikhil_c-_amd/csrc/mgx_launch.hpp b/multigrid_nikhil_c-_amd/csrc/mgx_launch.hpp
--- a/multigrid_nikhil_c-_amd/csrc/mgx_launch.hpp
+++ b/multigrid_nikhil_c-_amd/csrc/mgx_launch.hpp
@@ -5,6 +5,7 @@
 #include "mgx_pass_plan.hpp"
 
 #include <algorithm>
+#include <cstdio>
 
 namespace mgx {
 
@@ -101,6 +102,7 @@
     return false;
 }
 
+constexpr int kSeamDefaultMaxRows = 48;
 struct FoldArgs {
     const void* coarse_e = nullptr;
     void* coarse_b = nullptr;
@@ -109,6 +111,7 @@
     double* partial = nullptr;
     long cpitch = 0;
     int zero_in = 0;
+    int seam = 0;
     int row_lo = 0, row_hi = 0;
     CycleWin win{0, 0, 0, 0, 0, 0};
 };
@@ -147,12 +150,26 @@
     const bool bot_edge = (row_hi + K + EBOT - 1) > std::min(win.row_last, N - 1) || (PRE && ((row_hi + K + EBOT) >> 1) > win.crow_last);
     GeomKnobs kn = BL ? geom_knobs() : GeomKnobs();
     if (sizeof(T) == 4 && BL) kn.pair_min_rows = std::min(kn.pair_min_rows, env_int("MGX_PAIR_MIN_ROWS_F32", 100));
-    const CycleGeom g = cycle_geom_pick(row_lo, row_hi, strips, 2 * K + E, kTripSteps, R, auto_rows, BL, kn, top_edge, bot_edge);
+    CycleGeom g;
+    int seam = 0;
+    if constexpr (cycle_seam<T, K, PRE, POST, SM, AR>()) {
+        constexpr int ES = K + (POST == 1 ? 2 : (POST == 2 ? 1 : 0));
+        const bool whole = win.row_first == 0 && win.row_last == N && row_lo == 1 && row_hi == N;
+        const bool want = fa.seam >= 2 || (fa.seam == 1 && POST == 1);
+        if (want && whole && !(PRE != 0 && fa.zero_in) && seam_geom_pick(row_lo, row_hi, strips, 2 * K + E, ES, kTripSteps, R, auto_rows, kn, top_edge, bot_edge, &g, fa.seam >= 3))
+            seam = (fa.seam >= 2 || g.R <= kSeamDefaultMaxRows) ? 1 : 0;
+    }
+    if (!seam) g = cycle_geom_pick(row_lo, row_hi, strips, 2 * K + E, kTripSteps, R, auto_rows, BL, kn, top_edge, bot_edge);
     const int blocks = g.blocks;
+    if (BL && env_int("MGX_SEAM_LOG", 0)) {
+        const SeamCounts sc = seam_counts(strips, g.chunks, g.chunks_e, g.n_tall, g.n_short);
+        std::fprintf(stderr, "[mgx] deep pass N=%d K=%d pre=%d post=%d rows=[%d,%d) seam=%d seam_wgs=%d blocks=%d R=%d RB=%d Rf=%d Rl=%d tall=%d short=%d chunks=%d\n",
+                     N, K, PRE, POST, row_lo, row_hi, seam, seam ? sc.wt + sc.ws : 0, blocks, g.R, g.RB, g.Rf, g.Rl, g.n_tall, g.n_short, g.chunks);
+    }
     const T w = (fa.restrict_mode == MGX_RESTRICT_FW16) ? (T)0.0625 : (T)0.25;
     hipLaunchKernelGGL((k_jacobi_cycle<T, K, PRE, POST, SM, AR>), dim3(blocks), dim3(kBlock), 0, st, vin, b, vout,
                        (const T*)fa.coarse_e, (T*)fa.coarse_b, (T*)fa.coarse_zero, w, fa.partial, N, pitch, fa.cpitch,
-                       row_lo, row_hi, g.R, strips, g.chunks, g.Re, g.chunks_e, g.row_last0, g.Rl, g.RB, g.n_tall, g.n_short, g.Rf, c0, c1, fa.zero_in, win);
+                       row_lo, row_hi, g.R, strips, g.chunks, g.Re, g.chunks_e, g.row_last0, g.Rl, g.RB, g.n_tall, g.n_short, g.Rf, c0, c1, fa.zero_in, win, seam);
     return blocks;
 }
 
diff --git a/multigrid_nikhil_c-_amd/csrc/mgx_pass_plan.hpp b/multigrid_nikhil_c-_amd/csrc/mgx_pass_plan.hpp
--- a/multigrid_nikhil_c-_amd/csrc/mgx_pass_plan.hpp
+++ b/multigrid_nikhil_c-_amd/csrc/mgx_pass_plan.hpp
@@ -20,6 +20,7 @@
     int tile_wide; int tile_short_n;
     int plan_pre[8] = {0}; int n_pre = 0; int plan_post[8] = {0}; int n_post = 0; int plan_min_n = 8192;
     int arith = 0;
+    int seam = 1;
 };
 
 inline int fuse_rows_deep(int N, int rows)
@@ -66,6 +67,7 @@
     if (f.kmax < 1) f.kmax = 1;
     if (f.kmax > 10) f.kmax = 10;
     f.rows = env_int("MGX_FUSE_ROWS", 0);
+    f.seam = std::max(0, env_int("MGX_SEAM", 1));
     if (f.rows < 0) f.rows = 0;
     f.min_n = std::max(64, env_int("MGX_FUSE_MIN_N", 256));
     f.fold_kmax = std::max(1, std::min(f.kmax, env_int("MGX_FOLD_KMAX", 10)));
```

Result: slower. 1129 billion (-1.8%).
